# CookiePPP/cookietts

Hardware: AMD Instinct MI355X
Metric: audio samples/sec (22.05kHz) WaveGlow infer, 80×900 mel, 1/2/4/8 GPU; real-time factor (higher is better)
Workload: dtype f32; 1 GPU; WaveGlow full (12 flows, 512 WN ch, 8 groups, 8 layers) fp32 infer, batch 8 x (80x900) mel per GPU, sigma 0.6, random-init weights; batch_per_gpu=8, frames=900, parallelism=utterance-batch shard x1

## Files before the change

### cookietts_amd/_lib.py

```python
from __future__ import annotations

import ctypes as C
import os
import threading

import torch

from . import build as _build

_LOCK = threading.Lock()
_LIB = None


class WaveGlowConfig(C.Structure):
    _fields_ = [(n, C.c_int32) for n in (
        "n_mel_channels", "n_group", "n_flows", "n_early_every", "n_early_size",
        "win_length", "hop_length", "n_layers", "n_channels", "kernel_size", "cond_hidden", "speaker_embed_dim",
        "f32_gemm_mode")]


class StftConfig(C.Structure):
    _fields_ = [("filter_length", C.c_int32), ("hop_length", C.c_int32), ("win_length", C.c_int32),
                ("n_mel_channels", C.c_int32), ("clamp_val", C.c_float)]

# ... 253 lines not shown
    "ctts_waveflow_forward_f32": (C.c_int, [C.POINTER(WaveFlowConfig), _FP, _FP, _FP, _FP, C.c_float, C.c_int32, _FP, _FP, _FP, _FP,
                                            C.c_int32, C.c_int32, C.c_int32, _FP, C.c_size_t, _FP]),
    "ctts_waveflow_forward_cond_f32": (C.c_int, [C.POINTER(WaveFlowConfig), _FP, _FP, _FP, _FP, C.c_int32, C.c_int32, C.c_float,
                                                 C.c_int32, _FP, _FP, _FP, _FP, C.c_int32, C.c_int32, C.c_int32, _FP, C.c_size_t,
                                                 _FP]),
    "ctts_waveflow_abort_status": (C.c_int, [C.POINTER(WaveFlowConfig), C.c_int32, C.c_int32, _FP, C.c_size_t, _FP]),
    "ctts_wgax_packed_bytes": (C.c_size_t, [C.POINTER(WgaxConfig)]),
    "ctts_wgax_pack_flow": (C.c_int, [C.POINTER(WgaxConfig), C.c_int32, C.POINTER(WgaxFlowWeights), _FP, _FP]),
    "ctts_wgax_workspace_bytes": (C.c_size_t, [C.POINTER(WgaxConfig), C.c_int32, C.c_int64]),
    "ctts_wgax_inverse_f32": (C.c_int, [C.POINTER(WgaxConfig), _FP, _FP, _FP, C.c_int32, C.c_int32, C.c_int32, _FP,
                                        C.c_int32, C.c_int64, _FP, C.c_size_t, _FP]),
    "ctts_wgax_packed_f16_bytes": (C.c_size_t, [C.POINTER(WgaxConfig)]),
    "ctts_wgax_pack_flow_f16": (C.c_int, [C.POINTER(WgaxConfig), C.c_int32, C.POINTER(WgaxFlowWeights), _FP, _FP]),
    "ctts_wgax_workspace_f16_bytes": (C.c_size_t, [C.POINTER(WgaxConfig), C.c_int32, C.c_int64]),
    "ctts_wgax_inverse_f16": (C.c_int, [C.POINTER(WgaxConfig), _FP, _FP, _FP, C.c_int32, C.c_int32, C.c_int32, _FP,
                                        C.c_int32, C.c_int64, _FP, C.c_size_t, _FP]),
    "ctts_wgax_sep_packed_bytes": (C.c_size_t, [C.POINTER(WgaxConfig)]),
    "ctts_wgax_sep_pack_flow": (C.c_int, [C.POINTER(WgaxConfig), C.c_int32, C.POINTER(WgaxFlowWeights), C.POINTER(_FP),
                                          C.POINTER(_FP), _FP, _FP]),
    "ctts_wgax_sep_workspace_bytes": (C.c_size_t, [C.POINTER(WgaxConfig), C.c_int32, C.c_int64]),
    "ctts_wgax_sep_inverse_f32": (C.c_int, [C.POINTER(WgaxConfig), _FP, _FP, _FP, C.c_int32, C.c_int32, C.c_int32, _FP,
                                            C.c_int32, C.c_int64, _FP, C.c_size_t, _FP]),
    "ctts_depthwise_conv1d_f32": (C.c_int, [_FP, _FP, _FP, _FP] + [C.c_int32] * 7 + [_FP]),
    "ctts_hifigan_weight_floats": (C.c_size_t, [C.POINTER(HifiganConfig)]),
    "ctts_hifigan_packed_bytes": (C.c_size_t, [C.POINTER(HifiganConfig)]),
    "ctts_hifigan_pack_f32": (C.c_int, [C.POINTER(HifiganConfig), _FP, C.c_size_t, _FP, _FP]),
    "ctts_hifigan_workspace_bytes": (C.c_size_t, [C.POINTER(HifiganConfig), C.c_int32, C.c_int32]),
    "ctts_hifigan_forward_f32": (C.c_int, [C.POINTER(HifiganConfig), _FP, _FP, C.c_int32, _FP, C.c_int32, C.c_int32, _FP,
                                           C.c_size_t, _FP]),
    "ctts_hifigan_packed_f16_bytes": (C.c_size_t, [C.POINTER(HifiganConfig)]),
    "ctts_hifigan_pack_f16": (C.c_int, [C.POINTER(HifiganConfig), _FP, C.c_size_t, _FP, _FP]),
    "ctts_hifigan_workspace_f16_bytes": (C.c_size_t, [C.POINTER(HifiganConfig), C.c_int32, C.c_int32]),
    "ctts_hifigan_forward_f16": (C.c_int, [C.POINTER(HifiganConfig), _FP, _FP, C.c_int32, _FP, C.c_int32, C.c_int32, _FP,
                                           C.c_size_t, _FP]),
    "ctts_hifigan_packed_bf16x3_bytes": (C.c_size_t, [C.POINTER(HifiganConfig)]),
    "ctts_hifigan_pack_bf16x3": (C.c_int, [C.POINTER(HifiganConfig), _FP, C.c_size_t, _FP, _FP]),
    "ctts_hifigan_workspace_bf16x3_bytes": (C.c_size_t, [C.POINTER(HifiganConfig), C.c_int32, C.c_int32]),
    "ctts_hifigan_forward_bf16x3": (C.c_int, [C.POINTER(HifiganConfig), _FP, _FP, C.c_int32, _FP, C.c_int32, C.c_int32, _FP,
                                              C.c_size_t, _FP]),
    "ctts_replicate_halo_f32":(C.c_int, [_FP, C.c_int32, C.c_int32, C.c_int32, C.c_int32, C.c_int32, C.c_int32, _FP]),
    "ctts_embed_rows_f32": (C.c_int, [_FP, _FP, _FP, C.c_int32, C.c_int32, C.c_int32, C.c_int32, C.c_int32, C.c_int32,
                                      C.c_int32, _FP]),
    "ctts_scale_add_rows_f32": (C.c_int, [_FP, _FP, _FP, _FP, C.c_int32, C.c_int32, C.c_int32, C.c_int32, C.c_int32,
                                          _FP]),
    "ctts_deemphasis_f32": (C.c_int, [_FP, _FP, C.c_int32, C.c_int32, C.c_double, _FP]),
    "ctts_alignment_workspace_bytes": (C.c_size_t, [C.c_int32, C.c_int32, C.c_int32]),
    "ctts_alignment_metric_f32": (C.c_int, [_FP, _FP, _FP, C.c_int32, C.c_int32, C.c_int32, C.c_float, _FP, _FP,
                                            C.c_size_t, _FP]),
    "ctts_alignment_metric_masked_f32": (C.c_int, [_FP, _FP, _FP, _FP, C.c_int32, C.c_int32, C.c_int32, C.c_float, _FP, _FP,
                                                   C.c_size_t, _FP]),
    "ctts_first_over_thresh_f32": (C.c_int, [_FP, C.c_int32, C.c_int32, C.c_float, _FP, _FP]),
    "ctts_taco_loss_workspace_bytes": (C.c_size_t, [C.c_int32] * 4),
    "ctts_taco_loss_f32": (C.c_int, [C.POINTER(TacoLossParams)] + [_FP] * 13 + [C.c_int32] * 4 + [_FP, _FP, _FP, C.c_size_t,
                                                                                                  _FP]),
    "ctts_taco_loss_finalize_f32": (C.c_int, [C.POINTER(TacoLossParams)] + [_FP] * 9 + [C.c_int32] * 4 + [_FP, _FP, _FP,
                                                                                                          C.c_size_t, _FP]),
    "ctts_mel_error_packed_bytes": (C.c_size_t, [C.POINTER(MelErrorConfig)]),
    "ctts_mel_error_pack": (C.c_int, [C.POINTER(MelErrorConfig), C.c_int32, _FP, _FP, _FP, _FP]),
    "ctts_mel_error_workspace_bytes": (C.c_size_t, [C.POINTER(MelErrorConfig)] + [C.c_int32] * 3),
    "ctts_mel_error_f32": (C.c_int, [C.POINTER(MelErrorConfig)] + [_FP] * 6 + [C.c_int32] * 5 + [_FP] * 4 + [C.c_int32, _FP,
                                                                                                     C.c_size_t, _FP]),
    "ctts_mel_dtw_f32": (C.c_int, [_FP] * 6 + [C.c_int32] * 5 + [_FP]),
    "ctts_mel_dtw_generic_f32": (C.c_int, [_FP] * 6 + [C.c_int32] * 5 + [_FP]),
    "ctts_taco_stop_state_bytes": (C.c_size_t, [C.c_int32]),
    "ctts_taco_stop_reset": (C.c_int, [_FP, C.c_int32, C.c_int32, _FP]),
    "ctts_taco_stop_rule_f32": (C.c_int, [_FP, C.c_int32, C.c_int32, C.c_int32, C.c_int32, C.c_float, C.c_int32, _FP, _FP]),
    "ctts_retry_state_bytes": (C.c_size_t, [C.POINTER(RetryConfig)]),
    "ctts_retry_state_layout": (C.c_int, [C.POINTER(RetryConfig), C.POINTER(C.c_size_t)]),
    "ctts_retry_reset": (C.c_int, [C.POINTER(RetryConfig), _FP, _FP]),
    "ctts_retry_update_f32": (C.c_int, [C.POINTER(RetryConfig), _FP, _FP, _FP, _FP, _FP, _FP, C.c_int32, C.c_int32, _FP, _FP,
                                        _FP]),
    "ctts_retry_vocoder_batch_f32": (C.c_int, [C.POINTER(RetryConfig), _FP, _FP, C.c_int32, C.c_float, _FP]),
    "ctts_pcm16_concat": (C.c_int, [_FP, C.c_int32, _FP, C.c_int32, C.c_int64, C.c_int32, C.c_int32, _FP, C.c_int64, _FP,
                                    _FP]),
    "ctts_affine_rows_f32": (C.c_int, [_FP, C.c_int32, C.c_int32, C.c_int32, C.c_int32, C.c_int32, C.c_int32, C.c_float,
                                       C.c_float, _FP]),
    "ctts_vol_unscale_f32": (C.c_int, [_FP, C.c_int64, _FP]),
    "ctts_resample_rows_f32": (C.c_int, [_FP, _FP] + [C.c_int32] * 9 + [C.c_float, _FP]),
    "ctts_interleave_phases_f32": (C.c_int, [_FP, _FP] + [C.c_int32] * 10 + [_FP]),
    "ctts_last_gemm_loop": (C.c_int, []),
    "ctts_last_winograd_f43_width": (C.c_int, []),
    "ctts_tuning_reload": (C.c_int, []),
    "ctts_tuning_flags": (C.c_int, []),
    "ctts_profile_create": (C.c_int, [C.POINTER(C.c_void_p)]),
    "ctts_profile_bind": (C.c_int, [C.c_void_p]),
    "ctts_profile_collect": (C.c_int, [C.c_void_p, C.c_int32, C.POINTER(C.c_int64), C.POINTER(C.c_double)]),
    "ctts_profile_destroy": (C.c_int, [C.c_void_p]),
}

MODEL_GEMM_MODES = {None: 0, "default": 0, "f32": 1, "bf16x3": 2, "bf16x6": 3}
GEMM_MODES = {"f32": 1, "bf16x3": 2, "bf16x6": 3}
WG_OPT_COMPOSED_COND = 1


def model_gemm_mode(mode):
    try:
        return MODEL_GEMM_MODES[mode]
    except KeyError:
        raise ValueError(f"f32 GEMM mode {mode!r}: expected one of 'default', 'f32', 'bf16x3', 'bf16x6'") from None


def set_f32_gemm_mode(mode):
    if mode in (None, "default", "f32"):
        return "f32"
    raise RuntimeError(f"cookietts_amd.set_f32_gemm_mode({mode!r}): the process-wide default was removed; "
                       f"call model.set_f32_gemm_mode({mode!r}) on each model instead")


class Profile:

    def __init__(self):
        h = C.c_void_p()
        check(lib().ctts_profile_create(C.byref(h)), "ctts_profile_create")
        self._h = h

    def __enter__(self):
        check(lib().ctts_profile_bind(self._h), "ctts_profile_bind")
        return self

    def __exit__(self, *exc):
        check(lib().ctts_profile_bind(None), "ctts_profile_bind")
        return False

    bind = __enter__

    def unbind(self):
        self.__exit__()

    def collect(self, which):
        n, ms = C.c_int64(), C.c_double()
        check(lib().ctts_profile_collect(self._h, which, C.byref(n), C.byref(ms)), "ctts_profile_collect")
        return int(n.value), float(ms.value)

    def close(self):
        if self._h is not None and _LIB is not None:
            _LIB.ctts_profile_destroy(self._h)
        self._h = None

    def __del__(self):
        try:
            self.close()
        except Exception:
            pass


TUNING_BITS = {"CTTS_F32_NO_GLDS": 0, "CTTS_GEMM_NO_XCD_PAIR": 1, "CTTS_F32_WINOGRAD_FUSED_MIN": 2, "CTTS_BF16_NO_WIDE": 3, "CTTS_BF16_NO_PP": 4,
               "CTTS_F32_WINOGRAD_NO_FUSED": 5, "CTTS_F32_WINOGRAD_F43_MIN": 6, "CTTS_WF_NO_FUSE": 7,
               "CTTS_TACO_NO_FUSE": 8, "CTTS_F32_NO_SMALL": 9, "CTTS_F32_FORCE_SMALL": 10, "CTTS_F32_NO_SPLITK": 11, "CTTS_WF_NO_VEC_INTERP": 12,
               "CTTS_F32_NO_DEFER_SKIP": 13, "CTTS_WF_NO_REGION_SPLIT": 14, "CTTS_WF_NO_ROW_QUEUE": 15, "CTTS_WF_ROW_QUEUE_MIN": 16,
               "CTTS_WF_INJECT_ABORT": 17, "CTTS_WF_QUEUE_DEBUG": 18, "CTTS_F32_NO_ROUND_SPLIT": 19, "CTTS_BF16_PS": 20, "CTTS_BF16_NO_PS": 21,
               "CTTS_F32_WINOGRAD_NO_F43": 22,
               "CTTS_TACO_POLL_DELAY": 23, "CTTS_TACO_VALU": 24, "CTTS_UP_NO_MFMA": 25, "CTTS_F32_NO_WN_FOLD": 26, "CTTS_TACO_BG_NO_PIPE": 27,
               "CTTS_F32_NO_WINOGRAD": 28, "CTTS_F32_WINOGRAD_MIN": 29, "CTTS_F32_WINOGRAD_PLAIN": 30}
TUNING_BITS_EXT = {"CTTS_WF_FWD_ROWWISE": 31}


def tuning_reload():
    check(lib().ctts_tuning_reload(), "ctts_tuning_reload")


def tuning_active(name):
    bit = TUNING_BITS[name] if name in TUNING_BITS else TUNING_BITS_EXT[name]
    return bool(lib().ctts_tuning_flags() >> bit & 1)


PROF_WN_IN = 0
PROF_WN_RS = 1
PROF_WN_SKIP = 2
PROF_WN_IN0F = 3
PROF_WN_SKEND = 4
PROF_WN_RES_F = 5


class HipLibraryError(RuntimeError):
    pass


def lib_path():
    return _build.LIB_PATH


def lib():
    global _LIB
    if _LIB is not None:
        return _LIB
    with _LOCK:
        if _LIB is not None:
            return _LIB
        path = lib_path()
        if not os.path.exists(path):
            raise HipLibraryError(
                f"{path} is missing: build it with `python -m cookietts_amd.build` "
                "(or __graft_entry__.build()); there is no CPU fallback for the hot path")
        try:
            handle = C.CDLL(path)
        except OSError as e:
            raise HipLibraryError(f"cannot load {path}: {e}") from e
        for name, (res, args) in SIGNATURES.items():
            try:
                fn = getattr(handle, name)
            except AttributeError as e:
                raise HipLibraryError(f"{path} does not export {name}") from e
            fn.restype = res
            fn.argtypes = args
        if handle.ctts_abi_version() != 7:
            raise HipLibraryError(f"ABI version mismatch: library reports {handle.ctts_abi_version()}")
        _LIB = handle
    return _LIB


def last_error():
    msg = lib().ctts_last_error()
    return msg.decode(errors='replace') if msg else ''


def check(rc, what):
    if rc != 0:
        raise HipLibraryError(f"{what} failed (rc={rc}): {last_error()}")


def nbytes(fn, *args, what):
    n = fn(*args)
    if n == 0:
        raise HipLibraryError(f"{what}: {last_error()}")
    return n


def ptr(t):
    if t is None:
        return None
    return C.c_void_p(t.data_ptr())


def stream(device):
    return C.c_void_p(torch.cuda.current_stream(device).cuda_stream)
```

### cookietts_amd/csrc/gemm_f32.hip

```cpp
#include <atomic>
#include <cstdlib>
#include <mutex>

#include "gemm_f32.h"
#include "tuning.h"
#include "gemm_bf16.h"

namespace ctts {

typedef float f32x16 __attribute__((ext_vector_type(16)));

namespace {

constexpr int STAGE = GEMM_KC * (256 + 128);
constexpr int GEMM_GLDS_MAX_CHUNKS = 384;

__device__ __forceinline__ float fast_sigmoid(float u) {
    return __builtin_amdgcn_rcpf(1.0f + __builtin_amdgcn_exp2f(u * -1.4426950408889634f));
}
__device__ __forceinline__ float fast_tanh(float u) {
    return 1.0f - 2.0f * __builtin_amdgcn_rcpf(1.0f + __builtin_amdgcn_exp2f(u * 2.8853900817779268f));
}

typedef const __attribute__((address_space(1))) float* gfloat_ptr;
// ... 671 lines not shown
template <int EPI, bool GLDS>
void launch_shape_g(int bm, dim3 grid, hipStream_t stream, const GemmArgs& a) {
    const bool few = a.nseg <= 4;
    if (bm == 128) {
        if (few) hipLaunchKernelGGL((conv_gemm_f32_kernel<EPI, 1, 4, GLDS>), grid, dim3(256), 0, stream, a);
        else hipLaunchKernelGGL((conv_gemm_f32_kernel<EPI, 1, GEMM_MAX_SEG, GLDS>), grid, dim3(256), 0, stream, a);
    } else {
        if (few) hipLaunchKernelGGL((conv_gemm_f32_kernel<EPI, 2, 4, GLDS>), grid, dim3(256), 0, stream, a);
        else hipLaunchKernelGGL((conv_gemm_f32_kernel<EPI, 2, GEMM_MAX_SEG, GLDS>), grid, dim3(256), 0, stream, a);
    }
}

template <int EPI>
void launch_shape(int bm, dim3 grid, hipStream_t stream, const GemmArgs& a) {
    if (tuning().f32_no_glds || a.nch_total > GEMM_GLDS_MAX_CHUNKS) launch_shape_g<EPI, false>(bm, grid, stream, a);
    else if (gemm_split_level(a.gemm_mode) == 6) launch_shape_xs<EPI, 6>(bm, grid, stream, a);
    else if (gemm_split_level(a.gemm_mode) == 3) launch_shape_xs<EPI, 3>(bm, grid, stream, a);
    else launch_shape_g<EPI, true>(bm, grid, stream, a);
}

}

int get_gemm_f32_mode() { return gemm_f32_mode(); }
namespace { thread_local int t_last_loop = 0; }
void note_gemm_loop(int code) { t_last_loop = code; }
int last_gemm_loop() { return t_last_loop; }
int gemm_split_level(int m) {
    if (m == CTTS_GEMM_DEFAULT) m = gemm_f32_mode();
    if (m == CTTS_GEMM_BF16X3) return 3;
    if (m == CTTS_GEMM_BF16X6) return 6;
    return 0;
}
bool gemm_mode_is_split(int m) { return gemm_split_level(m) != 0; }

namespace {
std::mutex g_tune_mu;
Tuning g_tune{};
bool g_tune_loaded = false;
void load_tuning_locked() {
    auto on = [](const char* n) { return getenv(n) != nullptr; };
    auto num = [](const char* n, int d) { const char* v = getenv(n); return v ? atoi(v) : d; };
    g_tune.f32_no_glds = on("CTTS_F32_NO_GLDS");
    g_tune.f32_no_small = on("CTTS_F32_NO_SMALL");
    g_tune.f32_force_small = on("CTTS_F32_FORCE_SMALL");
    g_tune.f32_no_splitk = on("CTTS_F32_NO_SPLITK");
    g_tune.f32_no_round_split = on("CTTS_F32_NO_ROUND_SPLIT");
    g_tune.no_xcd_pair = on("CTTS_GEMM_NO_XCD_PAIR");
    g_tune.bf16_no_wide = on("CTTS_BF16_NO_WIDE");
    g_tune.bf16_no_pp = on("CTTS_BF16_NO_PP");
    g_tune.bf16_wide_min = num("CTTS_BF16_WIDE_MIN", 192);
    g_tune.bf16_ps = on("CTTS_BF16_PS");
    g_tune.bf16_no_ps = on("CTTS_BF16_NO_PS");
    g_tune.wf_no_fuse = on("CTTS_WF_NO_FUSE");
    g_tune.taco_no_fuse = on("CTTS_TACO_NO_FUSE");
    g_tune.taco_valu = on("CTTS_TACO_VALU");
    g_tune.up_no_mfma = on("CTTS_UP_NO_MFMA");
    g_tune.taco_bg_no_pipe = on("CTTS_TACO_BG_NO_PIPE");
    {
        static const int dflt[6] = {0x10000 | 36, 0x10000 | 96, 0x10000 | 12, 0x10000 | 20, 0x10000 | 8, 0x10000 | 8};
        int v[6];
        for (int i = 0; i < 6; ++i) v[i] = dflt[i];
        const char* e = getenv("CTTS_TACO_POLL_DELAY");
        if (e && sscanf(e, "%d,%d,%d,%d,%d,%d", v, v + 1, v + 2, v + 3, v + 4, v + 5) != 6)
            for (int i = 0; i < 6; ++i) v[i] = dflt[i];
        for (int i = 0; i < 6; ++i) g_tune.taco_poll_delay[i] = v[i] < 0 ? 0 : v[i];
        g_tune.taco_poll_delay_set = e != nullptr;
    }
    g_tune.wf_no_vec_interp = on("CTTS_WF_NO_VEC_INTERP");
    g_tune.wf_fwd_rowwise = on("CTTS_WF_FWD_ROWWISE");
    g_tune.wf_no_region_split = on("CTTS_WF_NO_REGION_SPLIT");
    g_tune.wf_no_row_queue = on("CTTS_WF_NO_ROW_QUEUE");
    g_tune.wf_row_queue_min = num("CTTS_WF_ROW_QUEUE_MIN", -1);
    g_tune.wf_inject_abort = num("CTTS_WF_INJECT_ABORT", 0);
    g_tune.wf_queue_debug = num("CTTS_WF_QUEUE_DEBUG", 0);
    g_tune.f32_no_defer_skip = on("CTTS_F32_NO_DEFER_SKIP");
    g_tune.f32_no_wn_fold = on("CTTS_F32_NO_WN_FOLD");
    g_tune.f32_no_winograd = on("CTTS_F32_NO_WINOGRAD");
    g_tune.f32_winograd_min = num("CTTS_F32_WINOGRAD_MIN", -1);
    g_tune.f32_winograd_plain = on("CTTS_F32_WINOGRAD_PLAIN");
    g_tune.f32_winograd_fused_min = num("CTTS_F32_WINOGRAD_FUSED_MIN", -1);
    g_tune.f32_winograd_no_fused = on("CTTS_F32_WINOGRAD_NO_FUSED");
    g_tune.f32_winograd_f43_min = num("CTTS_F32_WINOGRAD_F43_MIN", -1);
    g_tune.f32_winograd_no_f43 = on("CTTS_F32_WINOGRAD_NO_F43");
    g_tune.f32_cond_chain = on("CTTS_F32_COND_CHAIN");
    g_tune_loaded = true;
}
}

Tuning tuning() {
    std::lock_guard<std::mutex> lk(g_tune_mu);
    if (!g_tune_loaded) load_tuning_locked();
    return g_tune;
}
void reload_tuning() {
    std::lock_guard<std::mutex> lk(g_tune_mu);
    load_tuning_locked();
}

int gemm_check_args(int epi, const GemmArgs& a) {
    CTTS_CHECK_ARG(a.bm == 256 || a.bm == 128, "gemm: bm=%d", a.bm);
    CTTS_CHECK_ARG(gemm_mode_valid(a.gemm_mode), "gemm: f32_gemm_mode %d (0 default, 1 fp32 MFMA, 2 split bf16)", a.gemm_mode);
    const int bn = gemm_bn(a.bm);
    CTTS_CHECK_ARG(a.nseg >= 1 && a.nseg <= GEMM_MAX_SEG, "gemm: nseg=%d", a.nseg);
    int nch = 0;
    for (int s = 0; s < a.nseg; ++s) {
        CTTS_CHECK_ARG(a.seg[s].nch > 0 && a.seg[s].base, "gemm: empty segment %d", s);
        CTTS_CHECK_ARG(a.seg[s].shift >= -a.pad && a.seg[s].shift <= a.pad,
                       "gemm: shift %d exceeds halo %d", a.seg[s].shift, a.pad);
        nch += a.seg[s].nch;
    }
    CTTS_CHECK_ARG(nch == a.nch_total, "gemm: chunk count mismatch %d vs %d", nch, a.nch_total);
    if (a.interleave > 1) {
        CTTS_CHECK_ARG(a.interleave <= a.nseg, "gemm: interleave %d > nseg %d", a.interleave, a.nseg);
        for (int s = 1; s < a.interleave; ++s)
            CTTS_CHECK_ARG(a.seg[s].nch == a.seg[0].nch, "gemm: interleaved segments must have equal length");
    }
    CTTS_CHECK_ARG(a.a_nch_alloc == 0 || a.a_ch_off + a.nch_total <= a.a_nch_alloc, "gemm: A chunk window");
    CTTS_CHECK_ARG(a.ld % 4 == 0 && a.ntiles * bn + 2 * a.pad <= a.ld && a.L <= a.ntiles * bn,
                   "gemm: bad geometry ld=%d pad=%d L=%d ntiles=%d bn=%d", a.ld, a.pad, a.L, a.ntiles, bn);
    CTTS_CHECK_ARG(gemm_epi_is_pair(epi) || a.split % 32 == 0, "gemm: split %d not a multiple of 32", a.split);
    const int cpb = a.bm / 2;
    CTTS_CHECK_ARG(gemm_epi_is_pair(epi) ? (a.pairC > (a.MB - 1) * cpb && a.pairC <= a.MB * cpb)
                                         : (a.M > (a.MB - 1) * a.bm && a.M <= a.MB * a.bm),
                   "gemm: M=%d pairC=%d MB=%d bm=%d", a.M, a.pairC, a.MB, a.bm);
    CTTS_CHECK_ARG(a.dst_ld > 0 && a.dst0, "gemm: destination not set");
    CTTS_CHECK_ARG(a.addend_frames == 0 || ((epi == GEMM_EPI_GATE || epi == GEMM_EPI_GATEX) && a.addend && a.addend_frames <= a.addend_ld - a.addend_pad),
                   "gemm: interpolated addend needs the GATE epilogue (frames=%d)", a.addend_frames);
    CTTS_CHECK_ARG(a.gate >= 0 && a.gate < GATE_KINDS && (a.gate == 0 || epi == GEMM_EPI_GATE), "gemm: gate=%d with epilogue %d",
                   a.gate, epi);
    CTTS_CHECK_ARG((a.addend2 == nullptr && a.map_d == 0) ||
                       (epi == GEMM_EPI_GATE && a.gate == GATE_GTU && a.addend_frames == 0 && a.map_d >= 0 &&
                        (a.addend2 == nullptr || (a.addend && (a.addend2_sign == 1.0f || a.addend2_sign == -1.0f))) &&
                        (a.map_d == 0 || ((a.map_par == 0 || a.map_par == 1) && a.map_L > 0 && a.map_col0 >= 0))),
                   "gemm: second addend / mapped store need the GATE epilogue (epilogue %d, map_d=%d)", epi, a.map_d);
    CTTS_CHECK_ARG(epi != GEMM_EPI_GATE_RS ||
                       (a.bm == 128 && a.pairC <= 64 && a.MB == 1 && a.rs_wT && a.rs_bias && (a.rs_rows == 64 || a.rs_rows == 128)),
                   "gemm: fused res/skip needs bm=128, <= 64 channels, rs_wT / rs_bias and 64 or 128 res/skip rows");
    const int parts = a.parts > 1 ? a.parts : 1;
    CTTS_CHECK_ARG(a.parts >= 0 && a.parts <= 2 && (a.mseg == 0 || a.mseg == 2), "gemm: parts=%d mseg=%d", a.parts, a.mseg);
    if (parts > 1 || a.mseg) {
        CTTS_CHECK_ARG((epi == GEMM_EPI_SPLIT || (epi == GEMM_EPI_GATE && a.gate == GATE_GTU)) && a.bm == 256 && a.nseg <= 4 &&
                           a.interleave <= 1 && gemm_split_level(a.gemm_mode) == 0 && a.shape_blocks == 0 && a.addend_frames == 0,
                       "gemm: parts / mapped segment need the fp32 SPLIT or GATE launch of the 256-row shape (epilogue %d, nseg=%d)", epi, a.nseg);
        CTTS_CHECK_ARG(parts == 1 || epi != GEMM_EPI_SPLIT || (a.acc0 == 0 && a.src0 == nullptr && a.split >= a.M),
                       "gemm: a two-part SPLIT launch stores every row to dst0");
        CTTS_CHECK_ARG(parts == 1 || (long long)parts * a.ntiles * a.batch < (1ll << 31) / a.MB, "gemm: merged grid");
    }
    if (epi == GEMM_EPI_PHASE) {
        CTTS_CHECK_ARG(a.bm == 256 && a.nseg <= 4 && a.interleave <= 1 && gemm_split_level(a.gemm_mode) == 0 && parts == 1 && !a.mseg &&
                           a.shape_blocks == 0,
                       "gemm: the phase store needs the fp32 launch of the 256-row shape with <= 4 segments (nseg=%d)", a.nseg);
        CTTS_CHECK_ARG(a.phase >= 4 && a.phase <= 256 && (a.phase & (a.phase - 1)) == 0 && a.MB % a.phase == 0 && a.M == a.MB * a.bm,
                       "gemm: phase=%d MB=%d M=%d", a.phase, a.MB, a.M);
        CTTS_CHECK_ARG(a.dst_pad >= 0 && a.dst_pad % 4 == 0 && a.dst_ld % 4 == 0 && a.dst0_bstride % 4 == 0 &&
                           reinterpret_cast<uintptr_t>(a.dst0) % 16 == 0 && (long long)a.phase * a.L <= a.dst_ld - a.dst_pad,
                       "gemm: phase store dst_ld=%d dst_pad=%d phase=%d L=%d", a.dst_ld, a.dst_pad, a.phase, a.L);
    }
    if (a.mseg) {
        const GemmSeg& g = a.seg[1];
        CTTS_CHECK_ARG(epi == GEMM_EPI_GATE && a.nseg == 2 && a.map_d > 0 && a.map_d % 4 == 0 && a.map_col0 % 4 == 0 && a.mseg_pad >= 0 &&
                           a.mseg_pad % 4 == 0 && a.mseg_ld % 4 == 0 && a.mseg_ld - a.mseg_pad >= 4 && g.bstride % 4 == 0 &&
                           (parts == 1 || a.part_seg[1] % 4 == 0) && reinterpret_cast<uintptr_t>(g.base) % 16 == 0 && g.shift == 0 &&
                           g.mb_rows == 0,
                       "gemm: mapped segment d=%d col0=%d ld=%d pad=%d", a.map_d, a.map_col0, a.mseg_ld, a.mseg_pad);
    }
    return CTTS_OK;
// ... 119 lines not shown
```

### cookietts_amd/csrc/tuning.h

```cpp
#pragma once

namespace ctts {

struct Tuning {
    bool f32_no_glds;
    bool f32_no_small;
    bool f32_force_small;
    bool f32_no_splitk;
    bool f32_no_round_split;
    bool no_xcd_pair;
    bool bf16_no_wide;
    int bf16_wide_min;
    bool bf16_no_pp;
    bool bf16_ps;
    bool bf16_no_ps;
    bool wf_no_fuse;
    bool taco_poll_delay_set;
    int taco_poll_delay[6];
    bool taco_no_fuse;
    bool taco_bg_no_pipe;
    bool up_no_mfma;
    bool taco_valu;
    bool f32_no_defer_skip;
    bool f32_no_wn_fold;
    bool f32_no_winograd;
    int f32_winograd_min;
    bool f32_winograd_plain;
    int f32_winograd_fused_min;
    int f32_winograd_f43_min;
    bool f32_winograd_no_f43;
    bool f32_winograd_no_fused;
    bool f32_cond_chain;
    bool wf_no_region_split;
    bool wf_no_row_queue;
    int wf_row_queue_min;
    int wf_queue_debug;
    int wf_inject_abort;
    bool wf_fwd_rowwise;
    bool wf_no_vec_interp;
};

Tuning tuning();
void reload_tuning();

}
```

### cookietts_amd/csrc/waveglow_api.hip

```cpp
#include <mutex>
#include <vector>

#include "gemm_bf16.h"
#include "gemm_f32.h"
#include "tuning.h"
#include "waveglow_kernels.h"
#include "wn_winograd_layer.h"

namespace ctts {

static thread_local char g_err[512] = "";

void set_error(const char* fmt, ...) {
    va_list ap;
    va_start(ap, fmt);
    vsnprintf(g_err, sizeof(g_err), fmt, ap);
    va_end(ap);
}

namespace {

constexpr size_t ALIGN_F = 64;
inline size_t align_up(size_t v) { return (v + ALIGN_F - 1) / ALIGN_F * ALIGN_F; }
constexpr int A_TILE = GEMM_KC * GEMM_BM;

struct FlowDims { int n_rem, n_half, ch_off; };

struct Plan {
    ctts_waveglow_config c;
    int C, H, K0, n_in;
    int S;
    int nch0, nch1h, nch_in, nch_rs;
    int mb_in;
    int nch_in0f;
    std::vector<FlowDims> fd;
    size_t up_w, up_wp, up_b, cond0_A, cond0_b, cond1_A, cond1_b;
    size_t zero_b;
    bool up_mfma;
    bool cc;
    int ccP, ccJ, nch_cc;
    size_t cc_A, cc_b, cc_w10;
    struct Flow {
        size_t start_w, start_b, end_w, end_b, winv, spk_tab;
        std::vector<size_t> in_A, in_b, rs_A, rs_b;
        std::vector<size_t> res_A, res_b, skip_A, skip_b;
        size_t in0f_w, in0f_A, skend_W, skend_b;
        std::vector<size_t> wg_T2_A, wg_T3_A, wg_e_A, wg_o_A;
        size_t wg_dense;
        std::vector<size_t> wq_U_A[4], wq_e_A, wq_o_A;
    };
    std::vector<Flow> fl;
    size_t total;

    static constexpr int F32_SKIP_GROUP = 4;
    int mb_c() const { return (C + GEMM_BM - 1) / GEMM_BM; }
    int n_groups() const { return (c.n_layers + F32_SKIP_GROUP - 1) / F32_SKIP_GROUP; }
    int group_layers(int g) const { return g + 1 < n_groups() ? F32_SKIP_GROUP : c.n_layers - g * F32_SKIP_GROUP; }
    int rs_rows(int layer) const { return layer < c.n_layers - 1 ? 2 * C : C; }
    int rs_mb(int layer) const { return (rs_rows(layer) + GEMM_BM - 1) / GEMM_BM; }
};

int make_plan(const ctts_waveglow_config* cfg, Plan& p, int options = 0) {
    CTTS_CHECK_ARG(cfg != nullptr, "config is NULL");
    p.c = *cfg;
    CTTS_CHECK_ARG((options & ~CTTS_WG_OPT_COMPOSED_COND) == 0, "options=%d (CTTS_WG_OPT_*)", options);
    const bool want_cc = (options & CTTS_WG_OPT_COMPOSED_COND) != 0;
    const auto& c = p.c;
    CTTS_CHECK_ARG(c.n_flows >= 1 && c.n_layers >= 1 && c.n_layers <= 12, "n_flows=%d n_layers=%d", c.n_flows, c.n_layers);
    CTTS_CHECK_ARG(gemm_mode_valid(c.f32_gemm_mode), "f32_gemm_mode=%d (CTTS_GEMM_DEFAULT / _F32 / _BF16X3 / _BF16X6)", c.f32_gemm_mode);
    CTTS_CHECK_ARG(c.n_group >= 4 && c.n_group % 4 == 0 && c.n_group <= 16, "n_group=%d (4, 8, 12 or 16)", c.n_group);
    CTTS_CHECK_ARG(c.kernel_size == 3, "kernel_size=%d (only 3 built)", c.kernel_size);
    CTTS_CHECK_ARG(c.n_channels >= 128 && c.n_channels % 128 == 0, "n_channels=%d (multiple of 128)", c.n_channels);
    CTTS_CHECK_ARG(c.cond_hidden == GEMM_BM, "cond_hidden=%d (reference hard-codes 256)", c.cond_hidden);
    CTTS_CHECK_ARG(c.hop_length > 0 && c.win_length % c.hop_length == 0 && c.hop_length % c.n_group == 0,
                   "win=%d hop=%d n_group=%d", c.win_length, c.hop_length, c.n_group);
    CTTS_CHECK_ARG((c.n_mel_channels * c.n_group) % GEMM_KC == 0, "n_mel*n_group=%d not a multiple of 16",
                   c.n_mel_channels * c.n_group);
    CTTS_CHECK_ARG(c.n_early_every >= 1 && c.n_early_size >= 0 && c.n_early_size % 2 == 0, "early outputs");
    CTTS_CHECK_ARG(c.speaker_embed_dim >= 0 && c.speaker_embed_dim <= 1024, "speaker_embed_dim=%d", c.speaker_embed_dim);
    p.C = c.n_channels;
    p.H = c.cond_hidden;
    p.K0 = c.n_mel_channels * c.n_group;
    p.S = round_up(c.speaker_embed_dim, 32);
    CTTS_CHECK_ARG(p.S == 0 || p.K0 % 32 == 0, "multispeaker needs n_mel*n_group %% 32 == 0");
    p.nch0 = (p.K0 + p.S) / GEMM_KC;
    p.nch1h = p.H / GEMM_KC;
    p.nch_in = (c.kernel_size * p.C + p.H) / GEMM_KC;
    p.nch_rs = p.C / GEMM_KC;
    p.mb_in = 2 * p.C / GEMM_BM;
    p.nch_in0f = c.kernel_size + p.nch1h;
    int n_half = c.n_group / 2, n_rem = c.n_group;
    p.fd.resize(c.n_flows);
    for (int k = 0; k < c.n_flows; ++k) {
        if (k % c.n_early_every == 0 && k > 0) { n_half -= c.n_early_size / 2; n_rem -= c.n_early_size; }
        CTTS_CHECK_ARG(n_half >= 1 && n_rem == 2 * n_half, "flow %d: n_half=%d n_remaining=%d", k, n_half, n_rem);
        p.fd[k] = {n_rem, n_half, c.n_group - n_rem};
    }
    size_t o = 0;
    auto take = [&](size_t n) { size_t r = o; o = align_up(o + n); return r; };
    p.up_w = take((size_t)c.n_mel_channels * c.n_mel_channels * c.win_length);
    p.up_mfma = upsample_mfma_shape(c.n_mel_channels, c.win_length, c.hop_length, c.n_group);
    p.up_wp = p.up_mfma ? take((size_t)c.n_mel_channels * c.n_mel_channels * c.win_length) : 0;
    p.up_b = take(c.n_mel_channels);
    p.cond0_A = take((size_t)c.n_flows * p.nch0 * A_TILE);
    p.cond0_b = take((size_t)c.n_flows * GEMM_BM);
    p.cond1_A = take((size_t)c.n_flows * p.nch1h * A_TILE);
    p.cond1_b = take((size_t)c.n_flows * GEMM_BM);
    p.zero_b = take((size_t)p.mb_in * GEMM_BM);
    p.fl.resize(c.n_flows);
    for (int k = 0; k < c.n_flows; ++k) {
        auto& f = p.fl[k];
        f.start_w = take((size_t)p.C * p.fd[k].n_half);
        f.start_b = take(p.C);
        f.end_w = take((size_t)2 * p.fd[k].n_half * p.C);
        f.end_b = take(2 * p.fd[k].n_half);
        f.winv = take((size_t)p.fd[k].n_rem * p.fd[k].n_rem);
        f.spk_tab = take((size_t)CTTS_N_SPEAKERS * c.speaker_embed_dim);
        for (int i = 0; i < c.n_layers; ++i) {
            f.in_A.push_back(take((size_t)p.mb_in * p.nch_in * A_TILE));
            f.in_b.push_back(take((size_t)p.mb_in * GEMM_BM));
            f.rs_A.push_back(take((size_t)p.rs_mb(i) * p.nch_rs * A_TILE));
            f.rs_b.push_back(take((size_t)p.rs_mb(i) * GEMM_BM));
            f.res_A.push_back(i + 1 < c.n_layers ? take((size_t)p.mb_c() * p.nch_rs * A_TILE) : 0);
            f.res_b.push_back(i + 1 < c.n_layers ? take((size_t)p.mb_c() * GEMM_BM) : 0);
        }
        for (int gi = 0; gi < p.n_groups(); ++gi) {
            f.skip_A.push_back(take((size_t)p.mb_c() * p.group_layers(gi) * p.nch_rs * A_TILE));
            f.skip_b.push_back(take((size_t)p.mb_c() * GEMM_BM));
        }
        f.in0f_w = take((size_t)2 * p.C * FOLD_ROWS * c.kernel_size);
        f.in0f_A = take((size_t)p.mb_in * p.nch_in0f * A_TILE);
        f.skend_W = take((size_t)c.n_layers * p.C * 2 * p.fd[k].n_half);
        f.skend_b = take(2 * p.fd[k].n_half);
        for (int i = 0; i < c.n_layers; ++i) {
            f.wg_T2_A.push_back(take((size_t)p.mb_in * p.nch_rs * A_TILE));
            f.wg_T3_A.push_back(take((size_t)p.mb_in * p.nch_rs * A_TILE));
            f.wg_e_A.push_back(take((size_t)p.mb_in * (p.nch_rs + p.nch1h) * A_TILE));
            f.wg_o_A.push_back(take((size_t)p.mb_in * (p.nch_rs + p.nch1h) * A_TILE));
        }
        const bool f43 = wn_winograd_layer_f43_supported(p.C, p.H);
        for (int i = 0; f43 && i < c.n_layers; ++i) {
            for (auto& u : f.wq_U_A) u.push_back(take((size_t)p.mb_in * p.nch_rs * A_TILE));
            f.wq_e_A.push_back(take((size_t)p.mb_in * (p.nch_rs + p.nch1h) * A_TILE));
            f.wq_o_A.push_back(take((size_t)p.mb_in * (p.nch_rs + p.nch1h) * A_TILE));
        }
        f.wg_dense = take((size_t)(f43 ? 6 : 3) * 2 * p.C * p.C);
    }
    p.ccP = c.hop_length / c.n_group;
    p.ccJ = c.win_length / c.hop_length;
    p.nch_cc = p.ccJ * c.n_mel_channels / GEMM_KC;
    p.cc = want_cc && p.S == 0 && c.n_mel_channels % GEMM_KC == 0 && p.ccJ >= 1 && p.ccJ <= 4 && p.ccP >= 4 && p.ccP <= GEMM_BM &&
           (p.ccP & (p.ccP - 1)) == 0;
    p.cc_A = p.cc_b = p.cc_w10 = 0;
    if (p.cc) {
        p.cc_A = take((size_t)c.n_flows * p.ccP * p.nch_cc * A_TILE);
        p.cc_b = take((size_t)c.n_flows * p.ccP * GEMM_BM);
        p.cc_w10 = take((size_t)c.n_flows * 2 * p.H * p.K0);
    }
    p.total = o;
    return CTTS_OK;
}

struct Geom { int L, ld, pad, ntiles; };

int make_geom(const Plan& p, int frames, Geom& g) {
    CTTS_CHECK_ARG(frames >= 1, "frames=%d", frames);
    const long long T = (long long)frames * p.c.hop_length;
    g.L = (int)(T / p.c.n_group);
    int maxd = 1 << (p.c.n_layers - 1);
    g.pad = round_up(maxd > 128 ? maxd : 128, 32);
    g.ntiles = (g.L + GEMM_BN - 1) / GEMM_BN;
    g.ld = round_up(g.L, 256) + 2 * g.pad;
    return CTTS_OK;
}

struct PairGeom { int d, Lp, ntiles; };
PairGeom pair_geom(const Geom& g, int layer) {
    const int d = 1 << layer;
    const int Lp = (g.L + 2 * d - 1) / (2 * d) * d;
    return {d, Lp, (Lp + GEMM_BN - 1) / GEMM_BN};
}
int pair_ld(const Plan& p, const Geom& g) {
    int nt = 0;
    for (int i = 0; i < p.c.n_layers; ++i) nt = std::max(nt, pair_geom(g, i).ntiles);
    return nt * GEMM_BN;
}
PairGeom quad_geom(const Geom& g, int layer) {
    const int d = 1 << layer;
    const int Lq = (g.L + 4 * d - 1) / (4 * d) * d;
    return {d, Lq, (Lq + 63) / 64};
}
int quad_ld(const Plan& p, const Geom& g) {
    int nt = 0;
    for (int i = 0; i < p.c.n_layers; ++i) nt = std::max(nt, quad_geom(g, i).ntiles);
    return round_up(nt * 64, 128);
}
enum class InForm { Direct, WinogradSeparate, WinogradPaired, WinogradLayer, WinogradLayerF43 };

constexpr long long WINOGRAD_MIN_COLS = 28800;
constexpr long long WINOGRAD_FUSED_MIN_COLS = 28800;
constexpr long long WINOGRAD_F43_MIN_COLS = 28800;

InForm in_form(const Plan& p, const Geom& g, const Tuning& t) {
    auto long_enough = [&](int knob, long long cols) { return (long long)g.L >= (knob >= 0 ? knob : cols); };
    if (t.f32_no_winograd || gemm_split_level(p.c.f32_gemm_mode) != 0 || !long_enough(t.f32_winograd_min, WINOGRAD_MIN_COLS))
        return InForm::Direct;
    if (t.f32_winograd_plain || !gemm_f32_dma_staged(p.nch_rs + p.nch1h)) return InForm::WinogradSeparate;
    if (t.f32_winograd_no_fused || t.f32_no_glds || !wn_winograd_layer_supported(p.C, p.H) ||
        !long_enough(t.f32_winograd_fused_min, WINOGRAD_FUSED_MIN_COLS))
        return InForm::WinogradPaired;
    if (t.f32_winograd_no_f43 || !wn_winograd_layer_f43_supported(p.C, p.H) || !long_enough(t.f32_winograd_f43_min, WINOGRAD_F43_MIN_COLS))
        return InForm::WinogradLayer;
    return InForm::WinogradLayerF43;
}

bool cond_composed(const Plan& p, int frames, const Tuning& t) {
    if (!p.cc || t.f32_cond_chain || gemm_split_level(p.c.f32_gemm_mode) != 0) return false;
    const long long tiles_f = (frames + GEMM_BN - 1) / GEMM_BN, tiles_l = ((long long)frames * p.ccP + GEMM_BN - 1) / GEMM_BN;
    return tiles_f * p.ccP * p.ccJ * p.c.n_mel_channels < tiles_l * (p.K0 + p.H);
}
struct MelGeom { int ntiles, pad, ld; };
MelGeom mel_geom(int frames) {
    const int nt = (frames + GEMM_BN - 1) / GEMM_BN;
    return {nt, 4, nt * GEMM_BN + 8};
}

struct Workspace {
    float *audio, *spect, *spk, *h_tmp, *h_all, *x, *act, *out;
    float* melp;
    float* act_all;
    float* a16;
    float* skend;
    float *wgV, *wgT, *wgH;
    int ldp, ldq;
    size_t total;
};

void carve(const Plan& p, const Geom& g, int batch, float* base, InForm in, bool composed, Workspace& w) {
    size_t o = 0;
    auto take = [&](size_t n) { size_t r = o; o = align_up(o + n); return base ? base + r : nullptr; };
    const size_t B = batch;
    w.audio = take(B * p.c.n_group * g.L);
    w.spect = composed ? nullptr : take(B * p.K0 * g.ld);
    w.melp = composed ? take(B * p.c.n_mel_channels * mel_geom(g.L / p.ccP).ld) : nullptr;
    w.spk = take(B * p.c.n_flows * p.S * g.ld);
    w.h_tmp = composed ? nullptr : take(B * p.c.n_flows * p.H * g.ld);
    w.h_all = take(B * p.c.n_flows * p.H * g.ld);
    w.x = take(B * p.C * g.ld);
    w.act = take(B * p.C * g.ld);
    w.out = take(B * p.C * g.ld);
    w.act_all = take((size_t)std::min(p.c.n_layers, (int)Plan::F32_SKIP_GROUP) * B * p.C * g.ld);
    w.a16 = take(B * FOLD_ROWS * g.ld);
    w.skend = take(B * p.c.n_group * g.ld);
    w.wgV = w.wgT = w.wgH = nullptr;
    w.ldp = w.ldq = 0;
    if (in != InForm::Direct) {
        w.ldp = pair_ld(p, g);
        w.ldq = in == InForm::WinogradLayerF43 ? quad_ld(p, g) : 0;
        w.wgV = take(std::max((size_t)4 * w.ldp, (size_t)6 * w.ldq) * B * p.C);
        w.wgT = take((size_t)2 * B * 2 * p.C * w.ldp);
        w.wgH = take(std::max((size_t)2 * w.ldp, (size_t)4 * w.ldq) * B * p.H);
    }
    w.total = o;
}

struct Prof {
    std::mutex mu;
    std::vector<std::pair<hipEvent_t, hipEvent_t>> ev[CTTS_PROF_N];
    std::vector<std::pair<hipEvent_t, hipEvent_t>> pool;
};
thread_local Prof* t_prof = nullptr;

struct ProfScope {
    int which; hipStream_t s; hipEvent_t stop = nullptr; bool active = false;
    ProfScope(int which_, hipStream_t s_) : which(which_), s(s_) {
        Prof* pr = t_prof;
        if (!pr) return;
        std::lock_guard<std::mutex> lk(pr->mu);
        std::pair<hipEvent_t, hipEvent_t> e;
        if (!pr->pool.empty()) { e = pr->pool.back(); pr->pool.pop_back(); }
        else { if (hipEventCreate(&e.first) != hipSuccess || hipEventCreate(&e.second) != hipSuccess) return; }
        (void)hipEventRecord(e.first, s);
        stop = e.second;
        pr->ev[which].push_back(e);
        active = true;
    }
    ~ProfScope() { if (active) (void)hipEventRecord(stop, s); }
};

__global__ __launch_bounds__(256) void speaker_rows_kernel(const float* __restrict__ table, const int64_t* __restrict__ ids,
                                                           float* __restrict__ spk, int k, int n_flows, int S, int sdim,
                                                           int L, int ld, int pad) {
    const int n = blockIdx.x * 256 + threadIdx.x;
    const int e = blockIdx.y, b = blockIdx.z;
    if (n >= ld) return;
    float v = 0.f;
    if (e < sdim && n >= pad && n < pad + L) {
        const long long id = ids[b];
        v = (id >= 0 && id < CTTS_N_SPEAKERS) ? table[(size_t)id * sdim + e] : __builtin_nanf("");
    }
    spk[((size_t)b * n_flows * S + (size_t)k * S + e) * ld + n] = v;
}


__global__ __launch_bounds__(256) void cond_compose_w10_kernel(const float* __restrict__ w1, const float* __restrict__ w0,
                                                               double* __restrict__ w10, int H, int K0) {
    const int c = blockIdx.x * 256 + threadIdx.x, r = blockIdx.y;
    if (c >= K0) return;
    double s = 0.0;
    for (int h = 0; h < H; ++h) s += (double)w1[(size_t)r * H + h] * (double)w0[(size_t)h * K0 + c];
    w10[(size_t)r * K0 + c] = s;
}

__global__ __launch_bounds__(GEMM_BM) void cond_compose_A_kernel(const double* __restrict__ w10, const float* __restrict__ up_w,
                                                                 float* __restrict__ A, int n_mel, int G, int hop, int win, int P,
                                                                 int nch) {
    const int rl = threadIdx.x, kidx = blockIdx.x, m = blockIdx.y;
    const int r = m * (GEMM_BM / P) + rl / P, p = rl % P;
    const int j = kidx / n_mel, ci = kidx % n_mel;
    const float* u = up_w + (size_t)ci * n_mel * win + hop * j + G * p;
    const double* wr = w10 + (size_t)r * n_mel * G;
    double s = 0.0;
    for (int co = 0; co < n_mel; ++co)
        for (int q = 0; q < G; ++q) s += wr[co * G + q] * (double)u[(size_t)co * win + q];
    A[(((size_t)m * nch + kidx / GEMM_KC) * GEMM_KC + kidx % GEMM_KC) * GEMM_BM + rl] = (float)s;
}

__global__ __launch_bounds__(GEMM_BM) void cond_compose_bias_kernel(const float* __restrict__ w0, const float* __restrict__ b0,
                                                                    const float* __restrict__ w1, const float* __restrict__ b1,
                                                                    const float* __restrict__ up_b, float* __restrict__ bias, int K0,
                                                                    int G, int P) {
    __shared__ double t0[GEMM_BM];
    const int r = threadIdx.x;
    double s = b0[r];
    for (int c = 0; c < K0; ++c) s += (double)w0[(size_t)r * K0 + c] * (double)up_b[c / G];
    t0[r] = s;
    __syncthreads();
    s = b1[r];
    for (int h = 0; h < GEMM_BM; ++h) s += (double)w1[(size_t)r * GEMM_BM + h] * t0[h];
    const int HR = GEMM_BM / P;
    for (int p = 0; p < P; ++p) bias[(size_t)(r / HR) * GEMM_BM + (r % HR) * P + p] = (float)s;
}

__global__ __launch_bounds__(256) void mel_pad_kernel(const float* __restrict__ mel, float* __restrict__ melp, int frames, int ld, int pad) {
    const int n = blockIdx.x * 256 + threadIdx.x;
    const size_t row = (size_t)blockIdx.z * gridDim.y + blockIdx.y;
    if (n >= ld) return;
    const int f = n - pad;
    melp[row * ld + n] = f >= 0 && f < frames ? mel[row * frames + f] : 0.0f;
}

size_t fwd_mix_off(const Plan& p, int k) {
    size_t o = 0;
    for (int j = 0; j < k; ++j) o += align_up((size_t)p.fd[j].n_rem * p.fd[j].n_rem);
    return o;
}
int fwd_log_s_rows(const Plan& p, int k) {
    int r = 0;
    for (int j = 0; j < k; ++j) r += p.fd[j].n_half;
    return r;
}

struct FwdSums { double *ls_part, *z_part; int nblk_ls, nblk_z; size_t total; };

void carve_fwd(const Plan& p, const Geom& g, int batch, float* base, InForm in, bool composed, Workspace& w, FwdSums& f) {
    carve(p, g, batch, base, in, composed, w);
    f.nblk_ls = (g.L + 255) / 256;
    f.nblk_z = (int)(((long long)p.c.n_group * g.L + FWD_SUMSQ_CHUNK - 1) / FWD_SUMSQ_CHUNK);
    size_t o = w.total;
    auto take = [&](size_t doubles) { size_t r = o; o = align_up(o + 2 * doubles); return base ? reinterpret_cast<double*>(base + r) : nullptr; };
    f.ls_part = take((size_t)batch * p.c.n_flows * f.nblk_ls);
    f.z_part = take((size_t)batch * f.nblk_z);
    f.total = o;
}

int workspace_fits(const char* what, size_t have, size_t need) {
    if (need <= have) return CTTS_OK;
    set_error("%s: workspace %zu bytes < required %zu", what, have, need);
    return CTTS_E_WORKSPACE;
}

enum class StackForm { PerLayer, Deferred, Folded };

struct WnCall {
    Plan p; Geom g; Tuning t;
    const float* blob = nullptr;
    int batch = 0, frames = 0;
    hipStream_t s = nullptr;
    Workspace w{};
    FwdSums sums{};
    long long cstride = 0, hstride = 0;
    StackForm stack = StackForm::PerLayer;
    InForm in = InForm::Direct;
    bool composed = false;
    float* audio = nullptr;
    const float* h_all = nullptr;

    int begin(const ctts_waveglow_config* cfg, const void* packed, int batch_, int frames_, void* stream, int options = 0) {
        int rc = make_plan(cfg, p, options); if (rc) return rc;
        rc = make_geom(p, frames_, g); if (rc) return rc;
        t = tuning();
        blob = static_cast<const float*>(packed); batch = batch_; frames = frames_; s = as_stream(stream);
        cstride = (long long)p.C * g.ld;
        hstride = (long long)p.c.n_flows * p.H * g.ld;
        return CTTS_OK;
    }
    int take_workspace(const char* what, void* workspace, size_t workspace_bytes, bool forward) {
        in = in_form(p, g, t);
        stack = t.f32_no_defer_skip ? StackForm::PerLayer : t.f32_no_wn_fold ? StackForm::Deferred : StackForm::Folded;
        composed = cond_composed(p, frames, t);
        if (forward) carve_fwd(p, g, batch, static_cast<float*>(workspace), in, composed, w, sums);
        else carve(p, g, batch, static_cast<float*>(workspace), in, composed, w);
        audio = w.audio; h_all = w.h_all;
        return workspace_fits(what, workspace_bytes, (forward ? sums.total : w.total) * sizeof(float));
    }

    const float* h(int k) const { return h_all + (size_t)k * p.H * g.ld; }
    size_t act_stride() const { return (size_t)batch * p.C * g.ld; }
    float* act(int i) const { return stack == StackForm::PerLayer ? w.act : w.act_all + (size_t)(i % Plan::F32_SKIP_GROUP) * act_stride(); }
    bool group_ends(int i) const { return i == p.c.n_layers - 1 || (i + 1) % Plan::F32_SKIP_GROUP == 0; }
    bool in_place(int i) const { return in != InForm::WinogradSeparate && (1 << i) % 4 == 0; }
    size_t plane(int rows) const { return (size_t)batch * rows * w.ldp; }

    GemmArgs header() const {
        GemmArgs a{};
        a.gemm_mode = p.c.f32_gemm_mode;
        a.ld = g.ld; a.pad = g.pad; a.L = g.L; a.ntiles = g.ntiles; a.batch = batch;
        a.dst_ld = g.ld; a.dst_pad = g.pad;
        return a;
    }
    GemmArgs in_gemm(int k, int i) const {
        const auto& f = p.fl[k];
        const bool fold0 = stack == StackForm::Folded && i == 0;
        const int dil = 1 << i, nch = fold0 ? 1 : p.nch_rs;
        const float* taps = fold0 ? w.a16 : w.x;
        const long long tstride = fold0 ? (long long)FOLD_ROWS * g.ld : cstride;
        GemmArgs a = header();
        a.A = blob + (fold0 ? f.in0f_A : f.in_A[i]); a.bias = blob + f.in_b[i];
        a.nseg = 4; a.interleave = 3; a.nch_total = fold0 ? p.nch_in0f : p.nch_in; a.MB = p.mb_in;
        for (int tap = 0; tap < 3; ++tap) a.seg[tap] = {taps, tstride, nch, (tap - 1) * dil, 0, 0};
        a.seg[3] = {h(k), hstride, p.nch1h, 0, 0, 0};
        a.dst0 = act(i); a.dst0_bstride = cstride;
        a.M = 2 * p.C; a.pairC = p.C;
        return a;
    }
    GemmArgs behind(size_t A, size_t bias, int rows, const float* acts, int n, int split, bool acc1) const {
        GemmArgs a = header();
        a.A = blob + A; a.bias = blob + bias;
        a.nseg = n; a.nch_total = n * p.nch_rs; a.MB = (rows + GEMM_BM - 1) / GEMM_BM;
        for (int j = 0; j < n; ++j) a.seg[j] = {acts + (size_t)j * act_stride(), cstride, p.nch_rs, 0, 0, 0};
        a.M = rows; a.split = split;
        a.dst0 = w.x; a.dst0_bstride = cstride; a.acc0 = 1;
        a.dst1 = w.out; a.dst1_bstride = cstride; a.acc1 = acc1 ? 1 : 0;
        return a;
    }
    GemmArgs res(int k, int i) const { return behind(p.fl[k].res_A[i], p.fl[k].res_b[i], p.C, act(i), 1, p.C, false); }
    GemmArgs skip_group(int k, int gi) const { return behind(p.fl[k].skip_A[gi], p.fl[k].skip_b[gi], p.C, w.act_all, p.group_layers(gi), 0, gi > 0); }
    GemmArgs res_skip(int k, int i) const {
        return behind(p.fl[k].rs_A[i], p.fl[k].rs_b[i], p.rs_rows(i), act(i), 1, i == p.c.n_layers - 1 ? 0 : p.C, i > 0);
    }
    GemmArgs cond0(const float* spect, const float* spk, float* h_tmp) const {
        GemmArgs a = header();
        a.A = blob + p.cond0_A; a.bias = blob + p.cond0_b;
        a.nseg = 1; a.nch_total = p.nch0; a.MB = p.c.n_flows;
        a.seg[0] = {spect, (long long)p.K0 * g.ld, p.K0 / GEMM_KC, 0, 0, 0};
        if (p.S) {
            a.nseg = 2;
            a.seg[1] = {spk, (long long)p.c.n_flows * p.S * g.ld, p.S / GEMM_KC, 0, p.S, 0};
        }
        a.dst0 = h_tmp; a.dst0_bstride = hstride; a.acc0 = 0;
        a.dst1 = h_tmp; a.dst1_bstride = hstride; a.acc1 = 0;
        a.split = p.c.n_flows * GEMM_BM;
        a.M = p.c.n_flows * GEMM_BM;
        return a;
    }
    GemmArgs cond1(const float* spect, const float* spk, float* h_tmp, float* h_out) const {
        GemmArgs a = cond0(spect, spk, h_tmp);
        a.A = blob + p.cond1_A; a.bias = blob + p.cond1_b;
        a.nseg = 1; a.nch_total = p.nch1h;
        a.seg[0] = {h_tmp, hstride, p.nch1h, 0, GEMM_BM, 0};
        a.dst0 = h_out; a.dst1 = h_out;
        return a;
    }
    GemmArgs cond_composed_gemm(const float* melp, float* h_out) const {
        const MelGeom mg = mel_geom(frames);
        GemmArgs a{};
        a.gemm_mode = p.c.f32_gemm_mode;
        a.ld = mg.ld; a.pad = mg.pad; a.L = frames; a.ntiles = mg.ntiles; a.batch = batch;
        a.A = blob + p.cc_A; a.bias = blob + p.cc_b;
        a.nseg = p.ccJ; a.nch_total = p.nch_cc; a.MB = p.c.n_flows * p.ccP;
        for (int j = 0; j < p.ccJ; ++j)
            a.seg[j] = {melp, (long long)p.c.n_mel_channels * mg.ld, p.c.n_mel_channels / GEMM_KC, -j, 0, 0};
        a.M = a.MB * GEMM_BM; a.split = a.M;
        a.phase = p.ccP;
        a.dst0 = h_out; a.dst0_bstride = hstride; a.dst_ld = g.ld; a.dst_pad = g.pad;
        return a;
    }
    GemmArgs wg_header(int i) const {
        const PairGeom pg = pair_geom(g, i);
        GemmArgs a{};
        a.gemm_mode = p.c.f32_gemm_mode;
        a.ld = w.ldp; a.pad = 0; a.L = pg.Lp; a.ntiles = pg.ntiles; a.batch = batch; a.MB = p.mb_in;
        a.M = 2 * p.C;
        if (in == InForm::WinogradPaired) a.parts = 2;
        return a;
    }
    GemmArgs wg_T(int k, int i, int j) const {
        const auto& f = p.fl[k];
        GemmArgs a = wg_header(i);
        a.A = blob + (j == 0 ? f.wg_T2_A[i] : f.wg_T3_A[i]); a.bias = blob + p.zero_b;
        a.nseg = 1; a.nch_total = p.nch_rs;
        a.seg[0] = {w.wgV + (1 + j) * plane(p.C), (long long)p.C * w.ldp, p.nch_rs, 0, 0, 0};
        a.split = 2 * p.C;
        a.dst0 = w.wgT + j * plane(2 * p.C); a.dst0_bstride = (long long)2 * p.C * w.ldp; a.dst_ld = w.ldp; a.dst_pad = 0;
        if (a.parts == 2) {
            a.part_A = (long long)f.wg_T3_A[i] - (long long)f.wg_T2_A[i];
            a.part_seg[0] = (long long)plane(p.C);
            a.part_dst0 = (long long)plane(2 * p.C);
        }
        return a;
    }
    GemmArgs wg_gate(int k, int i, int j) const {
        const auto& f = p.fl[k];
        GemmArgs a = wg_header(i);
        a.A = blob + (j == 0 ? f.wg_e_A[i] : f.wg_o_A[i]); a.bias = blob + f.in_b[i];
        a.nseg = 2; a.nch_total = p.nch_rs + p.nch1h;
        a.seg[0] = {w.wgV + (j == 0 ? 0 : 3) * plane(p.C), (long long)p.C * w.ldp, p.nch_rs, 0, 0, 0};
        if (in_place(i)) {
            a.seg[1] = {h(k), hstride, p.nch1h, 0, 0, 0};
            a.mseg = 2; a.mseg_ld = g.ld; a.mseg_pad = g.pad;
        } else {
            a.seg[1] = {w.wgH + j * plane(p.H), (long long)p.H * w.ldp, p.nch1h, 0, 0, 0};
        }
        a.split = 0; a.pairC = p.C;
        a.dst0 = act(i); a.dst0_bstride = cstride; a.dst_ld = g.ld; a.dst_pad = g.pad;
        a.addend = w.wgT; a.addend2 = w.wgT + plane(2 * p.C); a.addend_bstride = (long long)2 * p.C * w.ldp;
        a.addend2_sign = j == 0 ? 1.0f : -1.0f;
        a.map_d = 1 << i; a.map_L = g.L; a.map_par = j;
        if (a.parts == 2) {
            a.part_A = (long long)f.wg_o_A[i] - (long long)f.wg_e_A[i];
            a.part_seg[0] = (long long)(3 * plane(p.C));
            a.part_seg[1] = in_place(i) ? 0 : (long long)plane(p.H);
        }
        return a;
    }
    WnWinogradLayerArgs wg_layer(int k, int i) const {
        const auto& f = p.fl[k];
        const bool f43 = in == InForm::WinogradLayerF43;
        const PairGeom sg = f43 ? quad_geom(g, i) : pair_geom(g, i);
        const int ldw = f43 ? w.ldq : w.ldp;
        WnWinogradLayerArgs a{};
        if (f43) {
            a.form = WNWG_F43;
            a.A_T2 = blob + f.wq_U_A[0][i]; a.A_T3 = blob + f.wq_U_A[1][i]; a.A_T4 = blob + f.wq_U_A[2][i]; a.A_T5 = blob + f.wq_U_A[3][i];
            a.A_e = blob + f.wq_e_A[i]; a.A_o = blob + f.wq_o_A[i];
        } else {
            a.A_T2 = blob + f.wg_T2_A[i]; a.A_T3 = blob + f.wg_T3_A[i]; a.A_e = blob + f.wg_e_A[i]; a.A_o = blob + f.wg_o_A[i];
        }
        a.bias = blob + f.in_b[i];
        a.V = w.wgV; a.vplane = (long long)batch * p.C * ldw;
        a.Hc = w.wgH; a.hplane = (long long)batch * p.H * ldw;
        a.h2 = h(k); a.h_bstride = hstride;
        a.act = act(i); a.act_bstride = cstride;
        a.C = p.C; a.H = p.H; a.batch = batch;
        a.ldp = ldw; a.Lp = sg.Lp; a.ntiles = sg.ntiles;
        a.d = sg.d; a.L = g.L; a.ld = g.ld; a.pad = g.pad;
        a.in_place = in_place(i);
        return a;
    }

    int gemm(int prof_slot, int epi, const GemmArgs& a) const {
        ProfScope ps(prof_slot, s);
        return launch_gemm_f32(epi, a, s);
    }
    int wg_transform(int k, int i) const {
        if (in == InForm::WinogradLayerF43) {
            const PairGeom qg = quad_geom(g, i);
            const int ncols = t.f32_no_small ? round_up(qg.ntiles * 64, 128) : qg.ntiles * 64;
            return launch_winograd_transform_quad(w.x, cstride, h(k), hstride, w.wgV, w.wgH, batch, p.C, p.H, qg.d, g.L, qg.Lp, g.ld, g.pad,
                                                  w.ldq, ncols, !in_place(i), s);
        }
        const PairGeom pg = pair_geom(g, i);
        return launch_winograd_transform(w.x, cstride, h(k), hstride, w.wgV, w.wgH, batch, p.C, p.H, pg.d, g.L, pg.Lp, g.ld, g.pad, w.ldp,
                                         pg.ntiles * GEMM_BN, !in_place(i), in != InForm::WinogradSeparate, s);
    }
    int in_layer(int k, int i) const {
        ProfScope ps(CTTS_PROF_WN_IN, s);
        if (stack == StackForm::Folded && i == 0) return gemm(CTTS_PROF_WN_IN0F, GEMM_EPI_GATE, in_gemm(k, i));
        int rc = in == InForm::Direct ? CTTS_OK : wg_transform(k, i);
        if (rc) return rc;
        switch (in) {
        case InForm::Direct:
            return launch_gemm_f32(GEMM_EPI_GATE, in_gemm(k, i), s);
        case InForm::WinogradLayer:
        case InForm::WinogradLayerF43:
            return launch_wn_winograd_layer(wg_layer(k, i), s);
        case InForm::WinogradSeparate:
        case InForm::WinogradPaired:
            const int np = in == InForm::WinogradPaired ? 1 : 2;
            for (int j = 0; j < np; ++j)
                if ((rc = launch_gemm_f32(GEMM_EPI_SPLIT, wg_T(k, i, j), s))) return rc;
            for (int j = 0; j < np; ++j)
                if ((rc = launch_gemm_f32(GEMM_EPI_GATE, wg_gate(k, i, j), s))) return rc;
        }
        return rc;
    }
    int start(int k, const float* a_in) const {
        const auto& f = p.fl[k];
        const auto& d = p.fd[k];
        return launch_wn_start(a_in, blob + f.start_w, blob + f.start_b, w.x, batch, p.C, p.c.n_group, d.ch_off, d.n_half, g.L, g.ld, g.pad, s);
    }
    int skip_end(int k, int gi, bool tail, float* wave, const CouplingForward* fwd) const {
        const auto& f = p.fl[k];
        const auto& d = p.fd[k];
        ProfScope ps(CTTS_PROF_WN_SKEND, s);
        return launch_skip_end(w.act_all, (long long)act_stride(), p.group_layers(gi),
                               blob + f.skend_W + (size_t)gi * Plan::F32_SKIP_GROUP * p.C * 2 * d.n_half, w.skend, gi == 0, tail,
                               blob + f.skend_b, blob + f.winv, audio, wave, batch, p.C, p.c.n_group, d.ch_off, d.n_half, g.L, g.ld,
                               g.pad, s, tail ? fwd : nullptr);
    }
    int flow_tail(int k, const float* out, float* a_io, float* wave, const CouplingForward* fwd) const {
        const auto& f = p.fl[k];
        const auto& d = p.fd[k];
        return launch_flow_tail(out, a_io, wave, blob + f.end_w, blob + f.end_b, blob + f.winv, batch, p.C, p.c.n_group, d.ch_off,
                                d.n_half, g.L, g.ld, g.pad, s, fwd);
    }

    int flow_folded(int k, float* wave, const CouplingForward* fwd) const {
        const auto& d = p.fd[k];
        int rc = start(k, audio);
        if (rc) return rc;
        if ((rc = launch_wn_start_ones(audio, w.a16, batch, p.c.n_group, d.ch_off, d.n_half, g.L, g.ld, g.pad, s))) return rc;
        for (int i = 0; i < p.c.n_layers; ++i) {
            const bool last = i == p.c.n_layers - 1;
            if ((rc = in_layer(k, i))) return rc;
            if (!last && (rc = gemm(CTTS_PROF_WN_RES_F, GEMM_EPI_SPLIT, res(k, i)))) return rc;
            if (group_ends(i) && (rc = skip_end(k, i / Plan::F32_SKIP_GROUP, last, wave, fwd))) return rc;
        }
        return CTTS_OK;
    }
    int stack_deferred(int k, const float* a_in) const {
        int rc = start(k, a_in);
        if (rc) return rc;
        for (int i = 0; i < p.c.n_layers; ++i) {
            if ((rc = in_layer(k, i))) return rc;
            if (i < p.c.n_layers - 1 && (rc = gemm(CTTS_PROF_WN_RS, GEMM_EPI_SPLIT, res(k, i)))) return rc;
            if (group_ends(i) && (rc = gemm(CTTS_PROF_WN_SKIP, GEMM_EPI_SPLIT, skip_group(k, i / Plan::F32_SKIP_GROUP)))) return rc;
        }
        return CTTS_OK;
    }
    int stack_per_layer(int k, const float* a_in) const {
        int rc = start(k, a_in);
        if (rc) return rc;
        for (int i = 0; i < p.c.n_layers; ++i) {
            if ((rc = in_layer(k, i))) return rc;
            if ((rc = gemm(CTTS_PROF_WN_RS, GEMM_EPI_SPLIT, res_skip(k, i)))) return rc;
        }
        return CTTS_OK;
    }
    int run_flow(int k, float* wave, const CouplingForward* fwd) const {
        if (stack == StackForm::Folded) return flow_folded(k, wave, fwd);
        const int rc = stack == StackForm::Deferred ? stack_deferred(k, audio) : stack_per_layer(k, audio);
        return rc ? rc : flow_tail(k, w.out, audio, wave, fwd);
    }
    int run_flow_forward(const float* fwd_blob, int k, const float* wave, float* log_s_flow, long long ls_bstride) const {
        const auto& d = p.fd[k];
        int rc = launch_flow_head_forward(fwd_blob + fwd_mix_off(p, k), wave, audio, batch, p.c.n_group, d.ch_off, d.n_rem, g.L, s);
        if (rc) return rc;
        const CouplingForward cf{log_s_flow, ls_bstride, sums.ls_part + (size_t)k * sums.nblk_ls, (long long)p.c.n_flows * sums.nblk_ls};
        return run_flow(k, nullptr, &cf);
    }

    int upsample(const float* mel, float* spect) const {
        return launch_upsample_squeeze(mel, blob + p.up_w, p.up_mfma ? blob + p.up_wp : nullptr, blob + p.up_b, spect, batch,
                                       p.c.n_mel_channels, frames, p.c.win_length, p.c.hop_length, p.c.n_group, g.ld, g.pad, s);
    }
    int speaker_rows(const int64_t* ids, float* spk) const {
        if (p.S == 0) return CTTS_OK;
// ... 376 lines not shown
    CTTS_CHECK_ARG(w && packed, "pack_flow: NULL pointer");
    hipStream_t s = as_stream(stream);
    float* blob = static_cast<float*>(packed);
    const auto& f = p.fl[k];
    const auto& d = p.fd[k];
    const int C = p.C, H = p.H, ks = p.c.kernel_size;
    auto d2d = [&](size_t off, const float* src, size_t n) -> int {
        CTTS_CHECK_ARG(src != nullptr, "pack_flow: NULL weight pointer");
        CTTS_CHECK_HIP(hipMemcpyAsync(blob + off, src, n * sizeof(float), hipMemcpyDeviceToDevice, s));
        return CTTS_OK;
    };
    if ((rc = d2d(f.start_w, w->start_w, (size_t)C * d.n_half))) return rc;
    if ((rc = d2d(f.start_b, w->start_b, C))) return rc;
    if ((rc = d2d(f.end_w, w->end_w, (size_t)2 * d.n_half * C))) return rc;
    if ((rc = d2d(f.end_b, w->end_b, 2 * d.n_half))) return rc;
    if ((rc = d2d(f.winv, w->w_inverse, (size_t)d.n_rem * d.n_rem))) return rc;
    CTTS_CHECK_ARG(w->cond_w[0] && w->cond_w[1] && w->cond_w[2] && w->cond_b[0] && w->cond_b[1] && w->cond_b[2],
                   "pack_flow: NULL cond weights");
    const int sdim = p.c.speaker_embed_dim;
    if ((rc = launch_pack_a(blob + p.cond0_A + (size_t)k * p.nch0 * A_TILE, w->cond_w[0], GEMM_BM, 1, p.nch0, 0, p.K0,
                            GEMM_EPI_SPLIT, C, H, 0, p.K0 + sdim, 1, s))) return rc;
    if (sdim) {
        if ((rc = launch_pack_a(blob + p.cond0_A + (size_t)k * p.nch0 * A_TILE, w->cond_w[0] + p.K0, GEMM_BM, 1, p.nch0,
                                p.K0, sdim, GEMM_EPI_SPLIT, C, H, 0, p.K0 + sdim, 1, s))) return rc;
        if ((rc = d2d(f.spk_tab, w->speaker_embed, (size_t)CTTS_N_SPEAKERS * sdim))) return rc;
    }
    if ((rc = launch_pack_bias(blob + p.cond0_b + (size_t)k * GEMM_BM, GEMM_BM, 1, w->cond_b[0], 0, nullptr, 0,
                               GEMM_EPI_SPLIT, C, H, s))) return rc;
    if ((rc = launch_pack_a(blob + p.cond1_A + (size_t)k * p.nch1h * A_TILE, w->cond_w[1], GEMM_BM, 1, p.nch1h, 0, H,
                            GEMM_EPI_SPLIT, C, H, 0, H, 1, s))) return rc;
    if ((rc = launch_pack_bias(blob + p.cond1_b + (size_t)k * GEMM_BM, GEMM_BM, 1, w->cond_b[1], 0, nullptr, 0,
                               GEMM_EPI_SPLIT, C, H, s))) return rc;
    for (int i = 0; i < p.c.n_layers; ++i) {
        CTTS_CHECK_ARG(w->in_w[i] && w->in_b[i] && w->rs_w[i] && w->rs_b[i], "pack_flow: NULL layer %d weights", i);
        for (int t = 0; t < ks; ++t)
            if ((rc = launch_pack_a(blob + f.in_A[i], w->in_w[i] + t, GEMM_BM, p.mb_in, p.nch_in, 0, C, GEMM_EPI_GATE, C,
                                    2 * C, 0, (long long)C * ks, ks, s, ks, t))) return rc;
        if ((rc = launch_pack_a(blob + f.in_A[i], w->cond_w[2], GEMM_BM, p.mb_in, p.nch_in, ks * C, H, GEMM_EPI_GATE, C,
                                2 * C, (long long)2 * C * i, H, 1, s))) return rc;
        if ((rc = launch_pack_bias(blob + f.in_b[i], GEMM_BM, p.mb_in, w->in_b[i], 0, w->cond_b[2], (long long)2 * C * i,
                                   GEMM_EPI_GATE, C, 2 * C, s))) return rc;
        const int rows = p.rs_rows(i);
        if ((rc = launch_pack_a(blob + f.rs_A[i], w->rs_w[i], GEMM_BM, p.rs_mb(i), p.nch_rs, 0, C, GEMM_EPI_SPLIT, C, rows,
                                0, C, 1, s))) return rc;
        if ((rc = launch_pack_bias(blob + f.rs_b[i], GEMM_BM, p.rs_mb(i), w->rs_b[i], 0, nullptr, 0, GEMM_EPI_SPLIT, C, rows,
                                   s))) return rc;
        const bool last = i == p.c.n_layers - 1;
        const int gi = i / Plan::F32_SKIP_GROUP, gj = i % Plan::F32_SKIP_GROUP;
        if (!last) {
            if ((rc = launch_pack_a(blob + f.res_A[i], w->rs_w[i], GEMM_BM, p.mb_c(), p.nch_rs, 0, C, GEMM_EPI_SPLIT, C, C,
                                    0, C, 1, s))) return rc;
            if ((rc = launch_pack_bias(blob + f.res_b[i], GEMM_BM, p.mb_c(), w->rs_b[i], 0, nullptr, 0, GEMM_EPI_SPLIT, C, C,
                                       s))) return rc;
        }
        if ((rc = launch_pack_a(blob + f.skip_A[gi], w->rs_w[i], GEMM_BM, p.mb_c(), p.group_layers(gi) * p.nch_rs, gj * C, C,
                                GEMM_EPI_SPLIT, C, C, last ? 0 : C, C, 1, s))) return rc;
        hipLaunchKernelGGL(skip_bias_kernel, dim3((p.mb_c() * GEMM_BM + 255) / 256), dim3(256), 0, s, blob + f.skip_b[gi],
                           w->rs_b[i] + (last ? 0 : C), C, p.mb_c() * GEMM_BM, gj == 0 ? 1 : 0);
        CTTS_CHECK_LAUNCH("skip_bias_f32");
    }
    auto pack_gate = [&](size_t A, const float* U, long long u_ld, int u_step, int i) -> int {
        const int nch = p.nch_rs + p.nch1h;
        const int rc = launch_pack_a(blob + A, U, GEMM_BM, p.mb_in, nch, 0, C, GEMM_EPI_GATE, C, 2 * C, 0, u_ld, u_step, s);
        return rc ? rc : launch_pack_a(blob + A, w->cond_w[2], GEMM_BM, p.mb_in, nch, C, H, GEMM_EPI_GATE, C, 2 * C, (long long)2 * C * i, H, 1, s);
    };
    for (int i = 0; i < p.c.n_layers; ++i) {
        float* dense = blob + f.wg_dense;
        const size_t dn = (size_t)2 * C * C;
        if ((rc = launch_winograd_g(w->in_w[i], dense, 2 * C, C, s))) return rc;
        if ((rc = launch_pack_a(blob + f.wg_T2_A[i], dense, GEMM_BM, p.mb_in, p.nch_rs, 0, C, GEMM_EPI_SPLIT, C, 2 * C, 0, C, 1, s))) return rc;
        if ((rc = launch_pack_a(blob + f.wg_T3_A[i], dense + dn, GEMM_BM, p.mb_in, p.nch_rs, 0, C, GEMM_EPI_SPLIT, C, 2 * C, 0, C, 1, s))) return rc;
        if ((rc = pack_gate(f.wg_e_A[i], w->in_w[i], (long long)C * ks, ks, i))) return rc;
        if ((rc = pack_gate(f.wg_o_A[i], dense + 2 * dn, C, 1, i))) return rc;
    }
    for (int i = 0; i < (f.wq_e_A.empty() ? 0 : p.c.n_layers); ++i) {
        float* dense = blob + f.wg_dense;
        const size_t dn = (size_t)2 * C * C;
        if ((rc = launch_winograd_g43(w->in_w[i], dense, 2 * C, C, s))) return rc;
        for (int j = 0; j < 4; ++j)
            if ((rc = launch_pack_a(blob + f.wq_U_A[j][i], dense + (1 + j) * dn, GEMM_BM, p.mb_in, p.nch_rs, 0, C, GEMM_EPI_SPLIT, C, 2 * C, 0, C, 1, s))) return rc;
        if ((rc = pack_gate(f.wq_e_A[i], dense, C, 1, i))) return rc;
        if ((rc = pack_gate(f.wq_o_A[i], dense + 5 * dn, C, 1, i))) return rc;
    }
    if ((rc = launch_fold_in0(w->in_w[0], w->start_w, w->start_b, blob + f.in0f_w, C, d.n_half, ks, s))) return rc;
    for (int t = 0; t < ks; ++t)
        if ((rc = launch_pack_a(blob + f.in0f_A, blob + f.in0f_w + t, GEMM_BM, p.mb_in, p.nch_in0f, 0, FOLD_ROWS, GEMM_EPI_GATE, C,
                                2 * C, 0, (long long)FOLD_ROWS * ks, ks, s, ks, t))) return rc;
    if ((rc = launch_pack_a(blob + f.in0f_A, w->cond_w[2], GEMM_BM, p.mb_in, p.nch_in0f, ks * FOLD_ROWS, H, GEMM_EPI_GATE, C,
                            2 * C, 0, H, 1, s))) return rc;
    return launch_fold_skend(w->rs_w, w->rs_b, w->end_w, w->end_b, blob + f.skend_W, blob + f.skend_b, C, p.c.n_layers, d.n_half, s);
}

size_t ctts_waveglow_packed_bytes_opt(const ctts_waveglow_config* cfg, int32_t options) {
    Plan p;
    if (make_plan(cfg, p, options)) return 0;
    return p.total * sizeof(float);
}

int ctts_waveglow_has_composed_cond(const ctts_waveglow_config* cfg) {
    Plan p;
    return make_plan(cfg, p, CTTS_WG_OPT_COMPOSED_COND) == CTTS_OK && p.cc ? 1 : 0;
}

int ctts_waveglow_pack_cond_composed(const ctts_waveglow_config* cfg, int32_t k, const ctts_waveglow_flow_weights* w, void* packed,
                                     void* stream) {
    Plan p;
    int rc = make_plan(cfg, p, CTTS_WG_OPT_COMPOSED_COND); if (rc) return rc;
    CTTS_CHECK_ARG(p.cc, "pack_cond_composed: this config has no composed conditioning (ctts_waveglow_has_composed_cond)");
    CTTS_CHECK_ARG(k >= 0 && k < p.c.n_flows, "pack_cond_composed: flow %d", k);
    CTTS_CHECK_ARG(w && packed && w->cond_w[0] && w->cond_w[1] && w->cond_b[0] && w->cond_b[1], "pack_cond_composed: NULL pointer");
    hipStream_t s = as_stream(stream);
    float* blob = static_cast<float*>(packed);
    const int H = p.H;
    double* w10 = reinterpret_cast<double*>(blob + p.cc_w10) + (size_t)k * H * p.K0;
    hipLaunchKernelGGL(cond_compose_w10_kernel, dim3((p.K0 + 255) / 256, H), dim3(256), 0, s, w->cond_w[1], w->cond_w[0], w10, H, p.K0);
    hipLaunchKernelGGL(cond_compose_A_kernel, dim3(p.ccJ * p.c.n_mel_channels, p.ccP), dim3(GEMM_BM), 0, s, w10, blob + p.up_w,
                       blob + p.cc_A + (size_t)k * p.ccP * p.nch_cc * A_TILE, p.c.n_mel_channels, p.c.n_group, p.c.hop_length,
                       p.c.win_length, p.ccP, p.nch_cc);
    hipLaunchKernelGGL(cond_compose_bias_kernel, dim3(1), dim3(GEMM_BM), 0, s, w->cond_w[0], w->cond_b[0], w->cond_w[1], w->cond_b[1],
                       blob + p.up_b, blob + p.cc_b + (size_t)k * p.ccP * GEMM_BM, p.K0, p.c.n_group, p.ccP);
    CTTS_CHECK_LAUNCH("cond_compose");
    return CTTS_OK;
}

size_t ctts_waveglow_workspace_bytes(const ctts_waveglow_config* cfg, int32_t batch, int32_t frames) {
    return ctts_waveglow_workspace_bytes_opt(cfg, batch, frames, 0);
}

size_t ctts_waveglow_workspace_bytes_opt(const ctts_waveglow_config* cfg, int32_t batch, int32_t frames, int32_t options) {
    Plan p; Geom g; Workspace w;
    if (make_plan(cfg, p, options) || make_geom(p, frames, g) || batch < 1) return 0;
    const Tuning t = tuning();
    carve(p, g, batch, nullptr, in_form(p, g, t), cond_composed(p, frames, t), w);
    return w.total * sizeof(float);
}

int ctts_upsample_squeeze_f32(const ctts_waveglow_config* cfg, const void* packed, const float* mel, float* spect,
                              int32_t batch, int32_t frames, void* stream) {
    WnCall c;
    const int rc = c.begin(cfg, packed, batch, frames, stream); if (rc) return rc;
    CTTS_CHECK_ARG(packed && mel && spect && batch >= 1, "upsample_squeeze: bad argument");
    return c.upsample(mel, spect);
}

int ctts_wn_cond_f32(const ctts_waveglow_config* cfg, const void* packed, const float* spect, const float* spk_rows,
                     float* h_tmp, float* h_all, int32_t batch, int32_t frames, void* stream) {
    WnCall c;
    const int rc = c.begin(cfg, packed, batch, frames, stream); if (rc) return rc;
    CTTS_CHECK_ARG(packed && spect && h_tmp && h_all && batch >= 1, "wn_cond: bad argument");
    return c.cond(spect, spk_rows, h_tmp, h_all);
}

size_t ctts_wn_cond_composed_scratch_bytes(const ctts_waveglow_config* cfg, int32_t batch, int32_t frames) {
    Plan p;
    if (make_plan(cfg, p, CTTS_WG_OPT_COMPOSED_COND) || !p.cc || batch < 1 || frames < 1) return 0;
    return (size_t)batch * p.c.n_mel_channels * mel_geom(frames).ld * sizeof(float);
}

int ctts_wn_cond_composed_f32(const ctts_waveglow_config* cfg, const void* packed, const float* mel, float* scratch, float* h_all,
                              int32_t batch, int32_t frames, void* stream) {
    WnCall c;
    const int rc = c.begin(cfg, packed, batch, frames, stream, CTTS_WG_OPT_COMPOSED_COND); if (rc) return rc;
    CTTS_CHECK_ARG(packed && mel && scratch && h_all && batch >= 1, "wn_cond_composed: bad argument");
    return c.cond_from_mel(mel, scratch, h_all);
}

// ... 53 lines not shown
    if (batch < 1) { set_error("forward_workspace_bytes: batch=%d", batch); return 0; }
    const Tuning t = tuning();
    carve_fwd(p, g, batch, nullptr, in_form(p, g, t), cond_composed(p, frames, t), w, f);
    return f.total * sizeof(float);
}

int ctts_waveglow_flow_forward_f32(const ctts_waveglow_config* cfg, const void* packed, const void* packed_fwd, int32_t flow,
                                   float* z, const float* wave, const float* h_all, float* log_s, double* sum_log_s,
                                   int32_t batch, int32_t frames, void* workspace, size_t workspace_bytes, void* stream) {
    WnCall c;
    int rc = c.begin(cfg, packed, batch, frames, stream); if (rc) return rc;
    CTTS_CHECK_ARG(flow >= 0 && flow < c.p.c.n_flows, "waveglow_flow_forward: flow %d", flow);
    CTTS_CHECK_ARG(packed && packed_fwd && z && h_all && workspace && batch >= 1, "waveglow_flow_forward: bad argument");
    CTTS_CHECK_ARG(wave == nullptr || flow == 0, "waveglow_flow_forward: only flow 0 reads the waveform (flow %d)", flow);
    if ((rc = c.take_workspace("waveglow_flow_forward", workspace, workspace_bytes, true))) return rc;
    c.audio = z; c.h_all = h_all;
    rc = c.run_flow_forward(static_cast<const float*>(packed_fwd), flow, wave, log_s, (long long)c.p.fd[flow].n_half * c.g.L);
    if (rc || !sum_log_s) return rc;
    const FwdSums& f = c.sums;
    return launch_sum_partials(f.ls_part + (size_t)flow * f.nblk_ls, (long long)c.p.c.n_flows * f.nblk_ls, 0, f.nblk_ls, sum_log_s, 1, 1,
                               batch, c.s);
}

int ctts_waveglow_forward_spk_f32(const ctts_waveglow_config* cfg, const void* packed, const void* packed_fwd, const float* mel,
                                  const float* audio, const int64_t* speaker_ids, float* z, float* log_s, double* sums,
                                  int32_t batch, int32_t frames, void* workspace, size_t workspace_bytes, void* stream) {
    WnCall c;
    int rc = c.begin(cfg, packed, batch, frames, stream); if (rc) return rc;
    const Plan& p = c.p;
    CTTS_CHECK_ARG(packed && packed_fwd && mel && audio && z && workspace && batch >= 1, "forward: bad argument");
    CTTS_CHECK_ARG(p.S == 0 || speaker_ids != nullptr, "multispeaker model (speaker_embed_dim=%d) needs speaker ids (glow.py:193)",
                   p.c.speaker_embed_dim);
    if ((rc = c.take_workspace("forward", workspace, workspace_bytes, true))) return rc;
    c.audio = z;
    if ((rc = c.conditioning(mel, speaker_ids))) return rc;
    const int L = c.g.L, S = fwd_log_s_rows(p, p.c.n_flows);
    for (int k = 0; k < p.c.n_flows; ++k) {
        float* ls = log_s ? log_s + (size_t)fwd_log_s_rows(p, k) * L : nullptr;
        rc = c.run_flow_forward(static_cast<const float*>(packed_fwd), k, k == 0 ? audio : nullptr, ls, (long long)S * L);
        if (rc) return rc;
    }
    if (!sums) return CTTS_OK;
    const FwdSums& f = c.sums;
    rc = launch_sum_partials(f.ls_part, (long long)p.c.n_flows * f.nblk_ls, f.nblk_ls, f.nblk_ls, sums, p.c.n_flows + 1, p.c.n_flows,
                             batch, c.s);
    if (rc) return rc;
    rc = launch_sumsq_partials(z, f.z_part, batch, (long long)p.c.n_group * L, f.nblk_z, c.s);
    if (rc) return rc;
    return launch_sum_partials(f.z_part, f.nblk_z, 0, f.nblk_z, sums + p.c.n_flows, p.c.n_flows + 1, 1, batch, c.s);
}

int ctts_waveglow_infer_f32(const ctts_waveglow_config* cfg, const void* packed, const float* mel,
                            const float* z_scaled, float* wave, int32_t batch, int32_t frames, void* workspace,
                            size_t workspace_bytes, void* stream) {
    return ctts_waveglow_infer_spk_f32(cfg, packed, mel, z_scaled, nullptr, wave, batch, frames, workspace,
                                       workspace_bytes, stream);
}

int ctts_waveglow_infer_spk_f32(const ctts_waveglow_config* cfg, const void* packed, const float* mel,
                                const float* z_scaled, const int64_t* speaker_ids, float* wave, int32_t batch,
                                int32_t frames, void* workspace, size_t workspace_bytes, void* stream) {
    return ctts_waveglow_infer_spk_f32_opt(cfg, packed, mel, z_scaled, speaker_ids, wave, batch, frames, workspace, workspace_bytes, 0,
                                           stream);
}

int ctts_waveglow_infer_spk_f32_opt(const ctts_waveglow_config* cfg, const void* packed, const float* mel,
                                    const float* z_scaled, const int64_t* speaker_ids, float* wave, int32_t batch,
                                    int32_t frames, void* workspace, size_t workspace_bytes, int32_t options, void* stream) {
    WnCall c;
    int rc = c.begin(cfg, packed, batch, frames, stream, options); if (rc) return rc;
    CTTS_CHECK_ARG(packed && mel && z_scaled && wave && workspace && batch >= 1, "infer: bad argument");
    if ((rc = c.take_workspace("infer", workspace, workspace_bytes, false))) return rc;
    CTTS_CHECK_HIP(hipMemcpyAsync(c.audio, z_scaled, (size_t)batch * c.p.c.n_group * c.g.L * sizeof(float), hipMemcpyDeviceToDevice, c.s));
    if ((rc = c.conditioning(mel, speaker_ids))) return rc;
    for (int k = c.p.c.n_flows - 1; k >= 0; --k)
        if ((rc = c.run_flow(k, k == 0 ? wave : nullptr, nullptr))) return rc;
    return CTTS_OK;
}


int ctts_last_gemm_loop(void) { return last_gemm_loop(); }
int ctts_last_winograd_f43_width(void) { return last_wn_winograd_f43_width(); }
int ctts_tuning_reload(void) { reload_tuning(); return CTTS_OK; }
int ctts_tuning_flags(void) {
    const Tuning t = tuning();
    return (t.f32_no_glds ? 1 : 0) | (t.no_xcd_pair ? 2 : 0) | (t.bf16_no_wide ? 8 : 0) | (t.bf16_no_pp ? 16 : 0) |
           (t.wf_no_fuse ? 128 : 0) | (t.taco_no_fuse ? 256 : 0) | (t.f32_no_small ? 512 : 0) | (t.f32_force_small ? 1024 : 0) |
           (t.f32_no_splitk ? 2048 : 0) | (t.wf_no_vec_interp ? 4096 : 0) | (t.f32_no_defer_skip ? 8192 : 0) |
           (t.wf_no_region_split ? 16384 : 0) | (t.wf_no_row_queue ? 32768 : 0) | (t.wf_row_queue_min >= 0 ? 65536 : 0) |
           (t.wf_inject_abort ? 131072 : 0) | (t.wf_queue_debug ? 262144 : 0) | (t.f32_no_round_split ? 524288 : 0) |
           (t.bf16_ps ? (1 << 20) : 0) | (t.bf16_no_ps ? (1 << 21) : 0) | (t.taco_poll_delay_set ? (1 << 23) : 0) |
           (t.taco_valu ? (1 << 24) : 0) | (t.up_no_mfma ? (1 << 25) : 0) | (t.f32_no_wn_fold ? (1 << 26) : 0) |
           (t.taco_bg_no_pipe ? (1 << 27) : 0) | (t.f32_no_winograd ? (1 << 28) : 0) | (t.f32_winograd_min >= 0 ? (1 << 29) : 0) |
           (t.f32_winograd_plain ? (1 << 30) : 0) | (t.f32_winograd_fused_min >= 0 ? 4 : 0) | (t.f32_winograd_no_fused ? 32 : 0) |
           (t.f32_winograd_f43_min >= 0 ? (1 << 6) : 0) | (t.f32_winograd_no_f43 ? (1 << 22) : 0) |
           (t.wf_fwd_rowwise ? (int)(1u << 31) : 0);
}

int ctts_profile_create(void** handle) {
    CTTS_CHECK_ARG(handle, "profile_create: NULL");
    *handle = new Prof();
    return CTTS_OK;
}

int ctts_profile_bind(void* handle) {
    t_prof = static_cast<Prof*>(handle);
    return CTTS_OK;
}

int ctts_profile_collect(void* handle, int32_t which, int64_t* launches, double* total_ms) {
    Prof* pr = static_cast<Prof*>(handle);
    CTTS_CHECK_ARG(pr && which >= 0 && which < CTTS_PROF_N && launches && total_ms, "profile_collect: bad argument");
    std::lock_guard<std::mutex> lk(pr->mu);
    double tot = 0.0;
    int64_t n = 0;
    for (auto& e : pr->ev[which]) {
        float ms = 0.f;
        CTTS_CHECK_HIP(hipEventSynchronize(e.second));
        CTTS_CHECK_HIP(hipEventElapsedTime(&ms, e.first, e.second));
        tot += ms; ++n;
        pr->pool.push_back(e);
    }
    pr->ev[which].clear();
    *launches = n; *total_ms = tot;
    return CTTS_OK;
}

int ctts_profile_destroy(void* handle) {
    Prof* pr = static_cast<Prof*>(handle);
    if (!pr) return CTTS_OK;
    if (t_prof == pr) t_prof = nullptr;
    {
        std::lock_guard<std::mutex> lk(pr->mu);
        for (int w = 0; w < CTTS_PROF_N; ++w)
            for (auto& e : pr->ev[w]) { (void)hipEventDestroy(e.first); (void)hipEventDestroy(e.second); }
        for (auto& e : pr->pool) { (void)hipEventDestroy(e.first); (void)hipEventDestroy(e.second); }
    }
    delete pr;
    return CTTS_OK;
}

static size_t packed_bf16_bytes_impl(const ctts_waveglow_config* cfg, int P) {
    Plan p; BfPlan q;
    if (make_plan(cfg, p)) return 0;
    if (p.C % BGEMM_KC != 0 || p.H % BGEMM_KC != 0) { set_error("bf16: channels must be multiples of 32"); return 0; }
    make_bf_plan(p, q, P);
    return q.total * sizeof(bf16_t);
}

static int pack_flow_bf16_impl(const ctts_waveglow_config* cfg, int32_t k, const ctts_waveglow_flow_weights* w,
                               void* packed_bf16, void* stream, int P, int f16 = 0) {
    Plan p; BfPlan q;
    int rc = make_plan(cfg, p); if (rc) return rc;
    CTTS_CHECK_ARG(k >= 0 && k < p.c.n_flows && w && packed_bf16, "pack_flow_bf16: bad argument");
    CTTS_CHECK_ARG(p.C % BGEMM_KC == 0 && p.H % BGEMM_KC == 0, "pack_flow_bf16: channels must be multiples of 32");
    CTTS_CHECK_ARG(!f16 || P == 1, "pack_flow: the split form exists for bf16 only");
    make_bf_plan(p, q, P, f16);
    CTTS_CHECK_ARG(q.nch_in <= BGEMM_MAX_CHUNKS && BF_SKIP_GROUP * q.nch_rs <= BGEMM_MAX_CHUNKS,
                   "pack_flow_bf16: K of %d chunks exceeds the chunk table", q.nch_in);
    hipStream_t s = as_stream(stream);
    bf16_t* bb = static_cast<bf16_t*>(packed_bf16);
    const int C = p.C, H = p.H, ks = p.c.kernel_size;
    CTTS_CHECK_ARG(w->cond_w[0] && w->cond_w[1] && p.K0 % BGEMM_KC == 0, "pack_flow_bf16: cond weights / n_mel*n_group %% 32");
    const int sdim = p.c.speaker_embed_dim;
    bf16_t* c0 = bb + q.cond0_A + (size_t)k * q.nch_c0 * BGEMM_KC * BGEMM_BM;
    bf16_t* c1 = bb + q.cond1_A + (size_t)k * q.nch_c1 * BGEMM_KC * BGEMM_BM;
// ... 163 lines not shown
```

### cookietts_amd/csrc/waveglow_kernels.h

```cpp
#pragma once

#include "common.h"
#include "gemm_f32.h"

namespace ctts {

int launch_fold_weightnorm(const float* v, const float* g, float* w, int out_ch, int fan, hipStream_t s);
int launch_pack_a(float* dst, const float* src, int bm, int MB, int nch_total, int k_off, int ksrc, int epi, int C, int M,
                  long long src_row_off, long long src_row_stride, int src_k_stride, hipStream_t s, int k_group = 1,
                  int k_member = 0);
int launch_pack_bias(float* dst, int bm, int MB, const float* src0, long long off0, const float* src1, long long off1,
                     int epi, int C, int M, hipStream_t s);
bool upsample_mfma_shape(int n_mel, int win, int hop, int G);
int launch_upsample_pack_mfma(const float* W, float* Wp, hipStream_t s);
int launch_upsample_squeeze(const float* mel, const float* W, const float* Wp, const float* bias, float* spect, int batch,
                            int n_mel, int F, int win, int hop, int G, int ld, int pad, hipStream_t s);
int launch_wn_start(const float* audio, const float* Ws, const float* bs, float* x, int batch, int C, int G,
                    int ch_off, int n_half, int L, int ld, int pad, hipStream_t s);
struct CouplingForward {
    float* log_s;
    long long ls_bstride;
    double* part;
    long long part_bstride;
};
constexpr int FWD_SUMSQ_CHUNK = 4096;
int launch_flow_tail(const float* out, float* audio, float* wave, const float* Wend, const float* bend,
                     const float* Winv, int batch, int C, int G, int ch_off, int n_half, int L, int ld, int pad,
                     hipStream_t s, const CouplingForward* fwd = nullptr);
int launch_flow_head_forward(const float* W, const float* wave, float* z, int batch, int G, int ch_off, int n_rem, int L,
                             hipStream_t s);
int launch_sumsq_partials(const float* z, double* part, int batch, long long n_item, int nblk, hipStream_t s);
int launch_sum_partials(const double* part, long long part_bstride, long long part_kstride, int n, double* out, int out_bstride,
                        int nk, int batch, hipStream_t s);

constexpr int FOLD_ROWS = 16;
int launch_fold_in0(const float* in_w, const float* Ws, const float* bs, float* dst, int C, int n_half, int ks, hipStream_t s);
int launch_fold_skend(const float* const* rs_w, const float* const* rs_b, const float* Wend, const float* bend, float* Wf,
                      float* bf, int C, int n_layers, int n_half, hipStream_t s);
int launch_wn_start_ones(const float* audio, float* a16, int batch, int G, int ch_off, int n_half, int L, int ld, int pad,
                         hipStream_t s);
int launch_skip_end(const float* act, long long act_stride, int nl, const float* Wf, float* acc, bool first, bool tail,
                    const float* bf, const float* Winv, float* audio, float* wave, int batch, int C, int G, int ch_off,
                    int n_half, int L, int ld, int pad, hipStream_t s, const CouplingForward* fwd = nullptr);

int launch_winograd_g(const float* in_w, float* dense, int rows, int C, hipStream_t s);
int launch_winograd_transform(const float* x, long long x_bstride, const float* h2, long long h_bstride, float* V, float* Hc,
                              int batch, int C, int H, int d, int L, int Lp, int ld, int pad, int ldp, int ncols, bool cond_rows,
                              bool vec_d2, hipStream_t s);

int launch_winograd_g43(const float* in_w, float* dense, int rows, int C, hipStream_t s);
int launch_winograd_transform_quad(const float* x, long long x_bstride, const float* h2, long long h_bstride, float* V, float* Hc,
                                   int batch, int C, int H, int d, int L, int Lq, int ld, int pad, int ldq, int ncols, bool cond_rows,
                                   hipStream_t s);

}
```

### cookietts_amd/csrc/waveglow_kernels.hip

```cpp
#include "waveglow_kernels.h"
#include "tuning.h"

namespace ctts {

namespace {

__global__ __launch_bounds__(256) void fold_weightnorm_kernel(const float* __restrict__ v,
                                                              const float* __restrict__ g,
                                                              float* __restrict__ w, int fan) {
    __shared__ float red[4];
    const int o = blockIdx.x;
    const float* vr = v + (size_t)o * fan;
    float s = 0.f;
    for (int i = threadIdx.x; i < fan; i += 256) { const float x = vr[i]; s = fmaf(x, x, s); }
#pragma unroll
    for (int off = 32; off > 0; off >>= 1) s += __shfl_xor(s, off);
    if ((threadIdx.x & 63) == 0) red[threadIdx.x >> 6] = s;
    __syncthreads();
    const float tot = red[0] + red[1] + red[2] + red[3];
    const float scale = g[o] / sqrtf(tot);
    float* wr = w + (size_t)o * fan;
    for (int i = threadIdx.x; i < fan; i += 256) wr[i] = vr[i] * scale;
}

// ... 530 lines not shown
    dense[2 * (size_t)n + idx] = (float)(-(w0 - w1 + w2) / 6.0);
    dense[3 * (size_t)n + idx] = (float)(w0 / 24.0 + w1 / 12.0 + w2 / 6.0);
    dense[4 * (size_t)n + idx] = (float)(w0 / 24.0 - w1 / 12.0 + w2 / 6.0);
    dense[5 * (size_t)n + idx] = in_w[(size_t)idx * 3 + 2];
}

template <int MODE>
__global__ __launch_bounds__(256) void winograd_transform_quad_kernel(const float* __restrict__ x, long long x_bstride,
                                                                      const float* __restrict__ h2, long long h_bstride,
                                                                      float* __restrict__ V, float* __restrict__ Hc, int C, int H,
                                                                      int d, int L, int Lq, int ld, int pad, int ldq, int ncols) {
    const int q4 = (blockIdx.x * 256 + threadIdx.x) * 4;
    if (q4 >= ncols) return;
    const int row = blockIdx.y, b = blockIdx.z, B = gridDim.z;
    const bool is_x = row < C;
    const float* src = is_x ? x + (size_t)b * x_bstride + (size_t)row * ld + pad
                            : h2 + (size_t)b * h_bstride + (size_t)(row - C) * ld + pad;
    float tap[6][4];
#pragma unroll
    for (int j = 0; j < 6; ++j)
#pragma unroll
        for (int e = 0; e < 4; ++e) tap[j][e] = 0.f;
    [[maybe_unused]] auto ld4 = [&](int t) { return (t >= 0 && t < L) ? *reinterpret_cast<const float4*>(src + t) : make_float4(0.f, 0.f, 0.f, 0.f); };
    if constexpr (MODE == 1) {
        if (q4 < Lq) {
            const int t0 = (q4 / d) * 4 * d + q4 % d;
#pragma unroll
            for (int j = 0; j < 6; ++j) {
                if (!is_x && (j == 0 || j == 5)) continue;
                const float4 v = ld4(t0 + (j - 1) * d);
                tap[j][0] = v.x; tap[j][1] = v.y; tap[j][2] = v.z; tap[j][3] = v.w;
            }
        }
    } else if constexpr (MODE == 2) {
        if (q4 < Lq) {
            float a[24];
#pragma unroll
            for (int u = 0; u < 6; ++u) {
                const float4 v = ld4(4 * q4 - 4 + 4 * u);
                a[4 * u] = v.x; a[4 * u + 1] = v.y; a[4 * u + 2] = v.z; a[4 * u + 3] = v.w;
            }
            const bool hi = q4 + 2 < Lq;
#pragma unroll
            for (int j = 0; j < 6; ++j) {
                tap[j][0] = a[4 + (j - 1) * 2]; tap[j][1] = a[5 + (j - 1) * 2];
                tap[j][2] = hi ? a[12 + (j - 1) * 2] : 0.f; tap[j][3] = hi ? a[13 + (j - 1) * 2] : 0.f;
            }
        }
    } else {
#pragma unroll
        for (int e = 0; e < 4; ++e) {
            const int q = q4 + e;
            const int t0 = (q / d) * 4 * d + q % d;
#pragma unroll
            for (int j = 0; j < 6; ++j) {
                const int t = t0 + (j - 1) * d;
                tap[j][e] = (q < Lq && t >= 0 && t < L && (is_x || (j >= 1 && j <= 4))) ? src[t] : 0.f;
            }
        }
    }
    if (is_x) {
        const size_t plane = (size_t)B * C * ldq;
        float* o = V + ((size_t)b * C + row) * ldq + q4;
        float v[6][4];
#pragma unroll
        for (int e = 0; e < 4; ++e) {
            const float x0 = tap[0][e], x1 = tap[1][e], x2 = tap[2][e], x3 = tap[3][e], x4 = tap[4][e], x5 = tap[5][e];
            const float s12 = x1 + x2, d12 = x1 - x2, s34 = x3 + x4, d34 = x3 - x4, d13 = x1 - x3, d24 = x2 - x4;
            v[0][e] = 4.f * x0 - 5.f * x2 + x4;
            v[1][e] = s34 - 4.f * s12;
            v[2][e] = 4.f * d12 - d34;
            v[3][e] = -2.f * d13 - d24;
            v[4][e] = 2.f * d13 - d24;
            v[5][e] = 4.f * x1 - 5.f * x3 + x5;
        }
#pragma unroll
        for (int j = 0; j < 6; ++j) *reinterpret_cast<float4*>(o + j * plane) = make_float4(v[j][0], v[j][1], v[j][2], v[j][3]);
    } else {
        const size_t plane = (size_t)B * H * ldq;
        float* o = Hc + ((size_t)b * H + (row - C)) * ldq + q4;
#pragma unroll
        for (int k = 0; k < 4; ++k) *reinterpret_cast<float4*>(o + k * plane) = make_float4(tap[k + 1][0], tap[k + 1][1], tap[k + 1][2], tap[k + 1][3]);
    }
}

template <int H>
__global__ __launch_bounds__(256) void wn_start_ones_kernel(const float* __restrict__ audio, float* __restrict__ a16, int G,
                                                            int ch_off, int L, int ld, int pad) {
    const int col = (blockIdx.x * 256 + threadIdx.x) * 4;
    const int b = blockIdx.z;
    if (col >= ld) return;
    const int n = col - pad;
    const bool in = n >= 0 && n < L;
    float* dst = a16 + (size_t)b * FOLD_ROWS * ld + col;
#pragma unroll
    for (int r = 0; r < FOLD_ROWS; ++r) {
        float4 v = make_float4(0.f, 0.f, 0.f, 0.f);
        if (in && r < H) v = *reinterpret_cast<const float4*>(audio + ((size_t)b * G + ch_off + r) * L + n);
        else if (in && r == H) v = make_float4(1.f, 1.f, 1.f, 1.f);
        *reinterpret_cast<float4*>(dst + (size_t)r * ld) = v;
    }
}

enum { SKEND_ACC = 0, SKEND_TAIL = 1, SKEND_FWD = 2 };
template <int H, int TAIL>
__global__ __launch_bounds__(256) void skip_end_kernel(const float* __restrict__ act, long long act_stride, int nl,
                                                       const float* __restrict__ Wf, float* __restrict__ acc, int first,
                                                       const float* __restrict__ bf, const float* __restrict__ Winv,
                                                       float* __restrict__ audio, float* __restrict__ wave,
                                                       int C, int G, int ch_off, int L, int ld, int pad, CouplingForward fw) {
    constexpr int E = 2 * H;
    constexpr int NG = E <= 4 ? 8 : E <= 8 ? 4 : 2;
    __shared__ __attribute__((aligned(16))) float part[3][E][256];
    __shared__ float sWinv[E * E];
    const int lane = threadIdx.x & 63;
    const int wv = threadIdx.x >> 6;
    const int b = blockIdx.y;
    const int n = blockIdx.x * 256 + lane * 4;
    if (TAIL == SKEND_TAIL && threadIdx.x < E * E) sWinv[threadIdx.x] = Winv[threadIdx.x];
    float4 e[E];
#pragma unroll
    for (int j = 0; j < E; ++j) e[j] = make_float4(0.f, 0.f, 0.f, 0.f);
    const int cq = C / 4;
    const int cbeg = __builtin_amdgcn_readfirstlane(wv * cq);
    for (int l = 0; l < nl; ++l) {
        const float* ob = act + (size_t)l * act_stride + (size_t)b * C * ld + pad + n;
        const float* wl = Wf + (size_t)l * C * E;
        for (int c = cbeg; c < cbeg + cq; c += NG) {
            float4 v[NG];
#pragma unroll
            for (int k = 0; k < NG; ++k) v[k] = *reinterpret_cast<const float4*>(ob + (size_t)(c + k) * ld);
#pragma unroll
            for (int k = 0; k < NG; ++k)
#pragma unroll
                for (int j = 0; j < E; ++j) {
                    const float w = wl[(c + k) * E + j];
                    e[j].x = fmaf(w, v[k].x, e[j].x); e[j].y = fmaf(w, v[k].y, e[j].y);
                    e[j].z = fmaf(w, v[k].z, e[j].z); e[j].w = fmaf(w, v[k].w, e[j].w);
                }
        }
    }
    if (wv > 0) {
#pragma unroll
        for (int j = 0; j < E; ++j) *reinterpret_cast<float4*>(&part[wv - 1][j][lane * 4]) = e[j];
    }
    __syncthreads();
    if (wv != 0 || (TAIL != SKEND_FWD && n >= L)) return;
    float* ab = acc + (size_t)b * E * ld + pad + n;
#pragma unroll
    for (int j = 0; j < E; ++j) {
#pragma unroll
        for (int q = 0; q < 3; ++q) {
            const float4 pv = *reinterpret_cast<const float4*>(&part[q][j][lane * 4]);
            e[j].x += pv.x; e[j].y += pv.y; e[j].z += pv.z; e[j].w += pv.w;
        }
        if (!first) {
            const float4 pv = *reinterpret_cast<const float4*>(ab + (size_t)j * ld);
            e[j].x += pv.x; e[j].y += pv.y; e[j].z += pv.z; e[j].w += pv.w;
        }
    }
    if constexpr (TAIL == SKEND_ACC) {
#pragma unroll
        for (int j = 0; j < E; ++j) *reinterpret_cast<float4*>(ab + (size_t)j * ld) = e[j];
    } else {
#pragma unroll
        for (int j = 0; j < E; ++j) {
// ... 125 lines not shown
    }
#undef CTTS_TAIL_CASE
    CTTS_CHECK_LAUNCH("flow_tail");
    return CTTS_OK;
}

int launch_fold_in0(const float* in_w, const float* Ws, const float* bs, float* dst, int C, int n_half, int ks, hipStream_t s) {
    CTTS_CHECK_ARG(n_half >= 1 && n_half < FOLD_ROWS, "fold_in0: n_half=%d", n_half);
    const int n = 2 * C * FOLD_ROWS * ks;
    hipLaunchKernelGGL(fold_in0_kernel, dim3((n + 255) / 256), dim3(256), 0, s, in_w, Ws, bs, dst, C, n_half, ks, 2 * C);
    CTTS_CHECK_LAUNCH("fold_in0");
    return CTTS_OK;
}

int launch_fold_skend(const float* const* rs_w, const float* const* rs_b, const float* Wend, const float* bend, float* Wf,
                      float* bf, int C, int n_layers, int n_half, hipStream_t s) {
    const int E = 2 * n_half;
    CTTS_CHECK_ARG(n_layers >= 1 && n_layers <= 12 && E <= 64, "fold_skend: n_layers=%d n_half=%d", n_layers, n_half);
    SkipBiasPtrs sb{};
    for (int i = 0; i < n_layers; ++i) {
        CTTS_CHECK_ARG(rs_w[i] && rs_b[i], "fold_skend: NULL layer %d weights", i);
        const int row_off = i < n_layers - 1 ? C : 0;
        sb.p[i] = rs_b[i];
        sb.row_off[i] = row_off;
        hipLaunchKernelGGL(fold_skend_w_kernel, dim3((C * E + 255) / 256), dim3(256), 0, s, Wend, rs_w[i], Wf + (size_t)i * C * E,
                           C, E, row_off);
    }
    hipLaunchKernelGGL(fold_skend_b_kernel, dim3(1), dim3(64), 0, s, Wend, bend, sb, n_layers, bf, C, E);
    CTTS_CHECK_LAUNCH("fold_skend");
    return CTTS_OK;
}

int launch_winograd_g(const float* in_w, float* dense, int rows, int C, hipStream_t s) {
    const int n = rows * C;
    hipLaunchKernelGGL(winograd_g_kernel, dim3((n + 255) / 256), dim3(256), 0, s, in_w, dense, n);
    CTTS_CHECK_LAUNCH("winograd_g");
    return CTTS_OK;
}

int launch_winograd_transform(const float* x, long long x_bstride, const float* h2, long long h_bstride, float* V, float* Hc,
                              int batch, int C, int H, int d, int L, int Lp, int ld, int pad, int ldp, int ncols, bool cond_rows,
                              bool vec_d2, hipStream_t s) {
    CTTS_CHECK_ARG(d >= 1 && Lp % d == 0 && (long long)Lp * 2 >= L && Lp <= ncols && ncols <= ldp && ncols % 4 == 0 && ldp % 4 == 0 &&
                       ld % 4 == 0 && pad % 4 == 0 && pad + L <= ld,
                   "winograd_transform: d=%d L=%d Lp=%d ncols=%d ldp=%d ld=%d pad=%d", d, L, Lp, ncols, ldp, ld, pad);
    dim3 grid((ncols / 4 + 255) / 256, cond_rows ? C + H : C, batch);
    if (d % 4 == 0 && L % 4 == 0)
        hipLaunchKernelGGL(winograd_transform_kernel<1>, grid, dim3(256), 0, s, x, x_bstride, h2, h_bstride, V, Hc, C, H, d, L, Lp,
                           ld, pad, ldp, ncols);
    else if (d == 2 && L % 4 == 0 && vec_d2)
        hipLaunchKernelGGL(winograd_transform_kernel<2>, grid, dim3(256), 0, s, x, x_bstride, h2, h_bstride, V, Hc, C, H, d, L, Lp,
                           ld, pad, ldp, ncols);
    else
        hipLaunchKernelGGL(winograd_transform_kernel<0>, grid, dim3(256), 0, s, x, x_bstride, h2, h_bstride, V, Hc, C, H, d, L, Lp,
                           ld, pad, ldp, ncols);
    CTTS_CHECK_LAUNCH("winograd_transform");
    return CTTS_OK;
}

int launch_winograd_g43(const float* in_w, float* dense, int rows, int C, hipStream_t s) {
    const int n = rows * C;
    hipLaunchKernelGGL(winograd_g43_kernel, dim3((n + 255) / 256), dim3(256), 0, s, in_w, dense, n);
    CTTS_CHECK_LAUNCH("winograd_g43");
    return CTTS_OK;
}

int launch_winograd_transform_quad(const float* x, long long x_bstride, const float* h2, long long h_bstride, float* V, float* Hc,
                                   int batch, int C, int H, int d, int L, int Lq, int ld, int pad, int ldq, int ncols, bool cond_rows,
                                   hipStream_t s) {
    CTTS_CHECK_ARG(d >= 1 && Lq % d == 0 && (long long)Lq * 4 >= L && Lq <= ncols && ncols <= ldq && ncols % 4 == 0 && ldq % 4 == 0 &&
                       ld % 4 == 0 && pad % 4 == 0 && pad + L <= ld && (!cond_rows || Hc != nullptr),
                   "winograd_transform_quad: d=%d L=%d Lq=%d ncols=%d ldq=%d ld=%d pad=%d", d, L, Lq, ncols, ldq, ld, pad);
    dim3 grid((ncols / 4 + 255) / 256, cond_rows ? C + H : C, batch);
    if (d % 4 == 0 && L % 4 == 0)
        hipLaunchKernelGGL(winograd_transform_quad_kernel<1>, grid, dim3(256), 0, s, x, x_bstride, h2, h_bstride, V, Hc, C, H, d, L, Lq,
                           ld, pad, ldq, ncols);
    else if (d == 2 && L % 4 == 0)
        hipLaunchKernelGGL(winograd_transform_quad_kernel<2>, grid, dim3(256), 0, s, x, x_bstride, h2, h_bstride, V, Hc, C, H, d, L, Lq,
                           ld, pad, ldq, ncols);
    else
        hipLaunchKernelGGL(winograd_transform_quad_kernel<0>, grid, dim3(256), 0, s, x, x_bstride, h2, h_bstride, V, Hc, C, H, d, L, Lq,
                           ld, pad, ldq, ncols);
    CTTS_CHECK_LAUNCH("winograd_transform_quad");
    return CTTS_OK;
}

int launch_wn_start_ones(const float* audio, float* a16, int batch, int G, int ch_off, int n_half, int L, int ld, int pad,
                         hipStream_t s) {
    CTTS_CHECK_ARG(L % 4 == 0 && ld % 4 == 0 && pad % 4 == 0, "wn_start_ones: L=%d ld=%d pad=%d", L, ld, pad);
    dim3 grid((ld / 4 + 255) / 256, 1, batch);
#define CTTS_ONES_CASE(H)                                                                                     \
    case H:                                                                                                   \
        hipLaunchKernelGGL(wn_start_ones_kernel<H>, grid, dim3(256), 0, s, audio, a16, G, ch_off, L, ld, pad); \
        break;
    switch (n_half) {
        CTTS_ONES_CASE(1) CTTS_ONES_CASE(2) CTTS_ONES_CASE(3) CTTS_ONES_CASE(4)
        CTTS_ONES_CASE(5) CTTS_ONES_CASE(6) CTTS_ONES_CASE(7) CTTS_ONES_CASE(8)
        default:
            set_error("wn_start_ones: n_half=%d unsupported (1..8)", n_half);
            return CTTS_E_ARG;
    }
#undef CTTS_ONES_CASE
    CTTS_CHECK_LAUNCH("wn_start_ones");
    return CTTS_OK;
}

int launch_skip_end(const float* act, long long act_stride, int nl, const float* Wf, float* acc, bool first, bool tail,
                    const float* bf, const float* Winv, float* audio, float* wave, int batch, int C, int G, int ch_off,
                    int n_half, int L, int ld, int pad, hipStream_t s, const CouplingForward* fwd) {
    CTTS_CHECK_ARG(fwd == nullptr || (tail && fwd->part != nullptr && wave == nullptr), "skip_end: forward direction on the tail pass only");
    const CouplingForward fw = fwd ? *fwd : CouplingForward{};
    CTTS_CHECK_ARG(L % 4 == 0 && C % 32 == 0 && ld % 4 == 0 && pad % 4 == 0 && nl >= 1, "skip_end: L=%d C=%d nl=%d", L, C, nl);
    CTTS_CHECK_ARG(acc != nullptr || (first && tail), "skip_end: a group after the first needs the accumulator");
    CTTS_CHECK_ARG(!tail || wave == nullptr || (ch_off == 0 && 2 * n_half == G && G % 4 == 0),
                   "skip_end: un-squeeze needs the full group (ch_off=%d n_half=%d G=%d)", ch_off, n_half, G);
    dim3 grid((L + 255) / 256, batch);
    const int fi = first ? 1 : 0;
#define CTTS_SKEND_CASE(H)                                                                                                \
    case H:                                                                                                               \
        if (fwd)                                                                                                          \
            hipLaunchKernelGGL((skip_end_kernel<H, SKEND_FWD>), grid, dim3(256), 0, s, act, act_stride, nl, Wf, acc, fi, bf, Winv, \
                               audio, wave, C, G, ch_off, L, ld, pad, fw);                                                \
        else if (tail)                                                                                                    \
            hipLaunchKernelGGL((skip_end_kernel<H, SKEND_TAIL>), grid, dim3(256), 0, s, act, act_stride, nl, Wf, acc, fi, bf, Winv, \
                               audio, wave, C, G, ch_off, L, ld, pad, fw);                                                \
        else                                                                                                              \
            hipLaunchKernelGGL((skip_end_kernel<H, SKEND_ACC>), grid, dim3(256), 0, s, act, act_stride, nl, Wf, acc, fi, bf, Winv, \
                               audio, wave, C, G, ch_off, L, ld, pad, fw);                                                \
        break;
    switch (n_half) {
        CTTS_SKEND_CASE(1) CTTS_SKEND_CASE(2) CTTS_SKEND_CASE(3) CTTS_SKEND_CASE(4)
        CTTS_SKEND_CASE(5) CTTS_SKEND_CASE(6) CTTS_SKEND_CASE(7) CTTS_SKEND_CASE(8)
        default:
            set_error("skip_end: n_half=%d unsupported (1..8)", n_half);
            return CTTS_E_ARG;
    }
#undef CTTS_SKEND_CASE
    CTTS_CHECK_LAUNCH("skip_end");
    return CTTS_OK;
}

int launch_flow_head_forward(const float* W, const float* wave, float* z, int batch, int G, int ch_off, int n_rem, int L,
                             hipStream_t s) {
    CTTS_CHECK_ARG(L % 4 == 0 && n_rem >= 2 && n_rem % 2 == 0 && ch_off >= 0 && ch_off + n_rem == G,
                   "flow_head_forward: L=%d n_rem=%d ch_off=%d G=%d", L, n_rem, ch_off, G);
    CTTS_CHECK_ARG(wave == nullptr || (ch_off == 0 && G % 4 == 0), "flow_head_forward: the squeeze needs the full group (ch_off=%d G=%d)",
                   ch_off, G);
    dim3 grid((L / 4 + 255) / 256, batch);
#define CTTS_HEAD_LAUNCH(EE, SQ) \
    hipLaunchKernelGGL((flow_head_forward_kernel<EE, SQ>), grid, dim3(256), 0, s, W, wave, z, G, ch_off, L)
#define CTTS_HEAD_CASE(EE)             \
    case EE:                           \
        CTTS_HEAD_LAUNCH(EE, false);   \
        break;
#define CTTS_HEAD_CASE_SQ(EE)                                                       \
    case EE:                                                                        \
        if (wave) CTTS_HEAD_LAUNCH(EE, true); else CTTS_HEAD_LAUNCH(EE, false);     \
        break;
    switch (n_rem) {
        CTTS_HEAD_CASE(2) CTTS_HEAD_CASE_SQ(4) CTTS_HEAD_CASE(6) CTTS_HEAD_CASE_SQ(8)
        CTTS_HEAD_CASE(10) CTTS_HEAD_CASE_SQ(12) CTTS_HEAD_CASE(14) CTTS_HEAD_CASE_SQ(16)
        default:
            set_error("flow_head_forward: n_rem=%d unsupported (2..16, even)", n_rem);
            return CTTS_E_ARG;
    }
#undef CTTS_HEAD_CASE_SQ
// ... 24 lines not shown
```

### cookietts_amd/csrc/wn_winograd_layer.h

```cpp
#pragma once

#include "common.h"
#include "gemm_f32.h"

namespace ctts {

constexpr int WNWG_MAX_CHUNKS = 320;
constexpr int WNWG_F23 = 0, WNWG_F43 = 1;

struct WnWinogradLayerArgs {
    const float *A_T2, *A_T3, *A_e, *A_o, *bias;
    const float *A_T4, *A_T5;
    const float* V; long long vplane;
    const float* Hc; long long hplane;
    const float* h2; long long h_bstride;
    float* act; long long act_bstride;
    int C, H, batch;
    int ldp, Lp, ntiles;
    int d, L, ld, pad;
    int in_place;
    int form;
    int kt, kt_total, b0, col0;
};

bool wn_winograd_layer_supported(int C, int H);
bool wn_winograd_layer_f43_supported(int C, int H);
int launch_wn_winograd_layer(const WnWinogradLayerArgs& a, hipStream_t stream);
int last_wn_winograd_f43_width();

}
```

### cookietts_amd/csrc/wn_winograd_layer.hip

```cpp
#include "wn_winograd_layer.h"
#include "tuning.h"

namespace ctts {

typedef float wg_f32x16 __attribute__((ext_vector_type(16)));
typedef unsigned wg_u32x4 __attribute__((ext_vector_type(4)));

namespace {

__device__ __forceinline__ float wg_sigmoid(float u) {
    return __builtin_amdgcn_rcpf(1.0f + __builtin_amdgcn_exp2f(u * -1.4426950408889634f));
}
__device__ __forceinline__ float wg_tanh(float u) {
    return 1.0f - 2.0f * __builtin_amdgcn_rcpf(1.0f + __builtin_amdgcn_exp2f(u * 2.8853900817779268f));
}

}

template <int NT, int F43, int KD, int TP>
__global__ __launch_bounds__(256, (F43 && NT == 2) ? 1 : 2) void wn_winograd_layer_f32_kernel(const WnWinogradLayerArgs a) {
    static_assert(KD == 1 || (KD == 2 && F43 && TP), "two chunks per stage: the F(4,3) form (its phases are whole stages, see the launcher)");
    constexpr int NI = F43 ? 4 : 2;
    constexpr int BN = 64 * NT;
    constexpr int A_ST = GEMM_KC * 128;
    constexpr int CST = A_ST + GEMM_KC * BN;
    constexpr int STG = KD * CST;
    constexpr int NP = 2 + NT;
    constexpr int TAB = 3 * STG;
    constexpr int BIAS = TAB + 4 * WNWG_MAX_CHUNKS;
    constexpr int UPR = BN / 4;
    constexpr int RPP = 64 / UPR;
    __shared__ __attribute__((aligned(16))) float lds[BIAS + 128];

    const int t = threadIdx.x;
    const int lane = t & 63;
    const int wave = __builtin_amdgcn_readfirstlane(t >> 6);
    const int wm = wave >> 1, wn = wave & 1;
    const int l31 = lane & 31, lhi = lane >> 5;

    const int ncb = a.C >> 6;
    const int jx = blockIdx.x >> 3;
    const int cb = jx % ncb;
    const int gt = (jx / ncb) * 8 + (blockIdx.x & 7);
    if (gt >= a.kt_total) return;
    const int b = a.b0 + gt / a.kt;
    const int n0 = a.col0 + (gt % a.kt) * BN;

    const int n1 = a.C / GEMM_KC, n2 = (a.C + a.H) / GEMM_KC, nh = a.H / GEMM_KC;
    const int c_e = NI * n1;
    int ps[NI + 1];
    ps[0] = c_e;
#pragma unroll
    for (int k = 0; k < NI; ++k) ps[k + 1] = ps[k] + (k == 0 || k == NI - 1 ? n2 : nh);
    const int nch = ps[NI];

    const int mb_t = (64 * cb) >> 8, loc_t = (64 * cb) & 255;
    const int mb_s = (a.C + 64 * cb) >> 8, loc_s = (a.C + 64 * cb) & 255;
    {
        uint4* tab = reinterpret_cast<uint4*>(lds + TAB);
        for (int c = t; c < nch; c += 256) {
            const float *ap, *bp;
            if (c < c_e) {
                const int ph = F43 ? c / n1 : (int)(c >= n1), loc = c - ph * n1;
                ap = (ph == 0 ? a.A_T2 : ph == 1 ? a.A_T3 : ph == 2 ? a.A_T4 : a.A_T5) + ((size_t)mb_t * n1 + loc) * (GEMM_KC * 256) + loc_t;
                bp = a.V + (1 + ph) * a.vplane + ((size_t)b * a.C + (size_t)loc * GEMM_KC) * a.ldp + n0;
            } else {
                int ph = 0;
#pragma unroll
                for (int k = 1; k < NI; ++k) ph += c >= ps[k];
                const bool last = ph == NI - 1;
                const int loc = c - ps[ph] + (ph == 0 || last ? 0 : n1);
                ap = (last ? a.A_o : a.A_e) + ((size_t)(cb >> 1) * n2 + loc) * (GEMM_KC * 256) + (cb & 1) * 128;
                if (loc < n1) bp = a.V + (last ? NI + 1 : 0) * a.vplane + ((size_t)b * a.C + (size_t)loc * GEMM_KC) * a.ldp + n0;
                else if (a.in_place) bp = a.h2 + (size_t)b * a.h_bstride + (size_t)(loc - n1) * GEMM_KC * a.ld;
                else bp = a.Hc + ph * a.hplane + ((size_t)b * a.H + (size_t)(loc - n1) * GEMM_KC) * a.ldp + n0;
            }
            const unsigned long long ua = reinterpret_cast<unsigned long long>(ap), ub = reinterpret_cast<unsigned long long>(bp);
            tab[c] = make_uint4((unsigned)ua, (unsigned)(ua >> 32), (unsigned)ub, (unsigned)(ub >> 32));
        }
        if (t < 128) lds[BIAS + t] = a.bias[cb * 128 + t];
    }

    unsigned offa_g[2], offa_s[2], offb[NT], offb_m[NI][NT];
    {
        const int col = (lane & 31) * 4;
        const long long delta = ((long long)(mb_s - mb_t) * n1) * (GEMM_KC * 256) + (loc_s - loc_t);
#pragma unroll
        for (int j = 0; j < 2; ++j) {
            const int krow = 2 * (wave + 4 * j) + (lane >> 5);
            offa_g[j] = (unsigned)((krow * 256 + col) * 4);
            offa_s[j] = (unsigned)((krow * 256 + (col < 64 ? (long long)col : col - 64 + delta)) * 4);
        }
        const int bcol = (lane % UPR) * 4;
#pragma unroll
        for (int j = 0; j < NT; ++j) {
            const int krow = (wave + 4 * j) * RPP + lane / UPR;
            offb[j] = (unsigned)(((size_t)krow * a.ldp + bcol) * 4);
#pragma unroll
            for (int k = 0; k < NI; ++k) offb_m[k][j] = 0;
            if (a.in_place) {
                const int q = n0 + bcol;
                const int te = (q / a.d) * (NI * a.d) + q % a.d;
                const int lim = (a.ld - a.pad - 4) & ~3;
#pragma unroll
                for (int k = 0; k < NI; ++k) offb_m[k][j] = (unsigned)(((size_t)krow * a.ld + a.pad + min(te + k * a.d, lim)) * 4);
            }
        }
    }
    int m_lo[NI];
#pragma unroll
    for (int k = 0; k < NI; ++k) m_lo[k] = a.in_place ? ps[k] + (k == 0 || k == NI - 1 ? n1 : 0) : 0x7fffffff;

    wg_f32x16 X[NI][2][NT];
#pragma unroll
    for (int k = 0; k < NI; ++k)
#pragma unroll
        for (int i = 0; i < 2; ++i)
#pragma unroll
            for (int j = 0; j < NT; ++j)
#pragma unroll
                for (int r = 0; r < 16; ++r) X[k][i][j][r] = 0.0f;
    __syncthreads();

    typedef __attribute__((address_space(3))) float* lds_fptr;
    typedef const __attribute__((address_space(1))) float* gfloat_ptr;
    typedef const __attribute__((address_space(1))) char* gbyte_ptr;
    const wg_u32x4* ctab = reinterpret_cast<const wg_u32x4*>(lds + TAB);
    wg_u32x4 tn_[KD];
    const unsigned tab_lds = (unsigned)reinterpret_cast<uintptr_t>((lds_fptr)(lds + TAB));
#define WNWG_TAB_ISSUE(c)                                                                                   \
    _Pragma("unroll") for (int j = 0; j < KD; ++j) asm volatile("ds_read_b128 %0, %1" : "=v"(tn_[j]) : "v"(tab_lds + 16u * (unsigned)((c) + j)));
#define WNWG_TAB_WAIT()                                                                                     \
    do {                                                                                                    \
        if constexpr (KD == 2) asm volatile("s_waitcnt lgkmcnt(0)" : "+v"(tn_[0]), "+v"(tn_[KD - 1]) : : "memory"); \
        else asm volatile("s_waitcnt lgkmcnt(0)" : "+v"(tn_[0]) : : "memory");                              \
    } while (0)
#define WNWG_ADDR(buf, c)                                                                                   \
    lds_fptr la_ = (lds_fptr)(lds + (buf) * STG + wave * 256);                                              \
    wg_u32x4 e_[KD];                                                                                        \
    _Pragma("unroll") for (int j = 0; j < KD; ++j) {                                                        \
        if constexpr (TP) e_[j] = tn_[j];                                                                   \
        else e_[j] = ctab[(c) + j];                                                                         \
    }                                                                                                       \
    const bool as_ = (c) < c_e;                                       \
    bool mk_[NI];                                                     \
    _Pragma("unroll") for (int k = 0; k < NI; ++k) mk_[k] = (c) >= m_lo[k] && (c) < ps[k + 1];
#define WNWG_BASES()                                                                                        \
// ... 82 lines not shown
    _Pragma("unroll") for (int nt = 0; nt < NT; ++nt) fb[r][nt] = (Bp)[((r) >> 3) * CST + (2 * ((r) & 7) + lhi) * BN + nt * 32];
#define WNWG_MM(Y, r)                                                                                       \
    _Pragma("unroll") for (int mt = 0; mt < 2; ++mt)                                                        \
        _Pragma("unroll") for (int nt = 0; nt < NT; ++nt)                                                   \
            Y[mt][nt] = __builtin_amdgcn_mfma_f32_32x32x2f32(fa[r][mt], fb[r][nt], Y[mt][nt], 0, 0, 0);
#define WNWG_R2(Y, r)                                                                                       \
    __builtin_amdgcn_sched_barrier(0);                                                                      \
    WNWG_RD((r) + 1, As, Bs)                                                                                \
    WNWG_MM(Y, r)                                                                                           \
    WNWG_PIECE(r);
#define WNWG_CHUNK2(Y)                                                                                      \
    {                                                                                                       \
        const float* As = lds + cur * STG + wm * 32 + l31;                                                  \
        const float* Bs = lds + cur * STG + A_ST + wn * (32 * NT) + l31;                                    \
        const int nx = cur == 2 ? 0 : cur + 1;                                                              \
        const float* An = lds + nx * STG + wm * 32 + l31;                                                   \
        const float* Bn = lds + nx * STG + A_ST + wn * (32 * NT) + l31;                                     \
        const int nb = cur >= 1 ? cur - 1 : 2;                      \
        const int cn = ch + 2 * KD < nch ? ch + 2 * KD : nch - KD;                                          \
        WNWG_ADDR(nb, cn)                                                                                   \
        __builtin_amdgcn_sched_barrier(0);                                                                  \
        WNWG_BASES()                                                                                        \
        WNWG_R2(Y, 0) WNWG_R2(Y, 1) WNWG_R2(Y, 2) WNWG_R2(Y, 3) WNWG_R2(Y, 4) WNWG_R2(Y, 5) WNWG_R2(Y, 6) WNWG_R2(Y, 7)   \
        WNWG_R2(Y, 8) WNWG_R2(Y, 9)                                                                         \
        WNWG_TAB_ISSUE(ch + 3 * KD < nch ? ch + 3 * KD : nch - KD)                                          \
        WNWG_R2(Y, 10) WNWG_R2(Y, 11) WNWG_R2(Y, 12) WNWG_R2(Y, 13) WNWG_R2(Y, 14)                          \
        __builtin_amdgcn_sched_barrier(0);                                                                  \
        WNWG_TAB_WAIT();                                                \
        WNWG_WAIT();                                         \
        __builtin_amdgcn_s_barrier();                                                                       \
        __builtin_amdgcn_sched_barrier(0);                                                                  \
        WNWG_RD(0, An, Bn)                                                                                  \
        WNWG_MM(Y, 15)                                                                                      \
        __builtin_amdgcn_sched_barrier(0);                                                                  \
        cur = nx;                                                                                           \
    }
#define WNWG_CHUNK(Y)                                                                                       \
    if constexpr (KD == 1) WNWG_CHUNK1(Y) else WNWG_CHUNK2(Y)
    if constexpr (KD == 2) {
        const float* As = lds + wm * 32 + l31;
        const float* Bs = lds + A_ST + wn * (32 * NT) + l31;
        WNWG_RD(0, As, Bs)
    }

    float* dst = a.act + (size_t)b * a.act_bstride + (size_t)(cb * 64 + wm * 32) * a.ld + a.pad;
    const float* bias = lds + BIAS + wm * 32;
#define WNWG_GATE(Y, par)                                                                                   \
    _Pragma("unroll") for (int nt = 0; nt < NT; ++nt) {                                                     \
        const int n = n0 + wn * (32 * NT) + nt * 32 + l31;                                                  \
        const int ns = (n / a.d) * (NI * a.d) + n % a.d + (par) * a.d;                                      \
        if (n < a.Lp && ns < a.L) {                                                                         \
            _Pragma("unroll") for (int r = 0; r < 16; ++r) {                                                \
                const int row = (r & 3) + 8 * (r >> 2) + 4 * lhi;                                           \
                const float u0 = Y[0][nt][r] + bias[row];                                                   \
                const float u1 = Y[1][nt][r] + bias[64 + row];                                              \
                dst[(size_t)row * a.ld + ns] = wg_tanh(u0) * wg_sigmoid(u1);                                \
            }                                                                                               \
        }                                                                                                   \
    }

#define WNWG_RUN(k, end) for (; ch < (end); ch += KD) WNWG_CHUNK(X[k])
#define WNWG_DRAIN()                                                                                        \
    asm volatile("s_waitcnt vmcnt(0)" ::: "memory");          \
    __builtin_amdgcn_s_barrier();
    int ch = 0;
    if constexpr (!F43) {
        WNWG_RUN(0, n1)
        WNWG_RUN(1, c_e)
#pragma unroll
        for (int i = 0; i < 2; ++i)
#pragma unroll
            for (int j = 0; j < NT; ++j)
#pragma unroll
                for (int r = 0; r < 16; ++r) {
                    const float s = X[0][i][j][r], dd = X[1][i][j][r];
                    X[0][i][j][r] = s + dd;
                    X[1][i][j][r] = s - dd;
                }
        WNWG_RUN(0, ps[1])
        WNWG_GATE(X[0], 0)
        WNWG_RUN(1, nch)
        WNWG_DRAIN()
        WNWG_GATE(X[1], 1)
    } else {
        WNWG_RUN(0, n1)
        WNWG_RUN(1, 2 * n1)
        WNWG_RUN(2, 3 * n1)
        WNWG_RUN(3, c_e)
#pragma unroll
        for (int i = 0; i < 2; ++i)
#pragma unroll
            for (int j = 0; j < NT; ++j)
#pragma unroll
                for (int r = 0; r < 16; ++r) {
                    if constexpr (NT == 2)
                        if (r == 0) asm volatile("" : "+a"(X[0][i][j]), "+a"(X[1][i][j]), "+a"(X[2][i][j]), "+a"(X[3][i][j]));
                    const float p1 = X[0][i][j][r], p2 = X[1][i][j][r], p3 = X[2][i][j][r], p4 = X[3][i][j][r];
                    const float sa = p1 + p2, sb = p1 - p2, sc = p3 + p4, se = p3 - p4;
                    X[0][i][j][r] = sa + sc;
                    X[1][i][j][r] = sb + 2.0f * se;
                    X[2][i][j][r] = sa + 4.0f * sc;
                    X[3][i][j][r] = sb + 8.0f * se;
                    if constexpr (NT == 2)
                        if (r == 15) asm volatile("" : "+a"(X[0][i][j]), "+a"(X[1][i][j]), "+a"(X[2][i][j]), "+a"(X[3][i][j]));
                }
#pragma unroll
        for (int k = 0; k < NI; ++k)
#pragma unroll
            for (int i = 0; i < 2; ++i) {
                if constexpr (NT == 2) { asm volatile("" : "+a"(X[k][i][0])); asm volatile("" : "+a"(X[k][i][1])); }
                else asm volatile("" : "+v"(X[k][i][0]));
            }
        WNWG_RUN(0, ps[1])
        WNWG_GATE(X[0], 0)
        WNWG_RUN(1, ps[2])
        WNWG_GATE(X[1], 1)
        WNWG_RUN(2, ps[3])
        WNWG_GATE(X[2], 2)
        WNWG_RUN(3, nch)
        WNWG_DRAIN()
        WNWG_GATE(X[3], 3)
    }
#undef WNWG_DRAIN
#undef WNWG_RUN
#undef WNWG_GATE
#undef WNWG_CHUNK
#undef WNWG_CHUNK2
#undef WNWG_R2
#undef WNWG_MM
#undef WNWG_RD
#undef WNWG_CHUNK1
#undef WNWG_REGION
#undef WNWG_MFMA
#undef WNWG_READ_FRAGS
#undef WNWG_WAIT
#undef WNWG_PIECE
#undef WNWG_BASES
#undef WNWG_TAB_WAIT
#undef WNWG_TAB_ISSUE
#undef WNWG_ADDR
}

bool wn_winograd_layer_supported(int C, int H) {
    return C >= 128 && C % 128 == 0 && H > 0 && H % GEMM_KC == 0 && 2 * (C / GEMM_KC) + 2 * ((C + H) / GEMM_KC) <= WNWG_MAX_CHUNKS;
}

bool wn_winograd_layer_f43_supported(int C, int H) {
    return wn_winograd_layer_supported(C, H) && 4 * (C / GEMM_KC) + 2 * ((C + H) / GEMM_KC) + 2 * (H / GEMM_KC) <= WNWG_MAX_CHUNKS;
}

namespace {
thread_local int t_last_f43_width = 0;

template <int NT, int F43, int KD, int TP>
int launch_wnwg_shape(WnWinogradLayerArgs a, int kt, long long kt_total, hipStream_t stream) {
    a.kt = kt;
    a.kt_total = (int)kt_total;
    const long long blocks = 8ll * (a.C / 64) * ((kt_total + 7) / 8);
    CTTS_CHECK_ARG(blocks > 0 && blocks < (1ll << 31) && kt_total < (1ll << 31), "wn_winograd_layer: grid %lld", blocks);
    hipLaunchKernelGGL((wn_winograd_layer_f32_kernel<NT, F43, KD, TP>), dim3((unsigned)blocks), dim3(256), 0, stream, a);
    CTTS_CHECK_LAUNCH("wn_winograd_layer");
    return CTTS_OK;
}

}

int last_wn_winograd_f43_width() { return t_last_f43_width; }

int launch_wn_winograd_layer(const WnWinogradLayerArgs& a_in, hipStream_t stream) {
    WnWinogradLayerArgs a = a_in;
    CTTS_CHECK_ARG(wn_winograd_layer_supported(a.C, a.H), "wn_winograd_layer: C=%d H=%d", a.C, a.H);
    CTTS_CHECK_ARG(a.A_T2 && a.A_T3 && a.A_e && a.A_o && a.bias && a.V && a.act && a.batch >= 1, "wn_winograd_layer: operand not set");
    const bool f43 = a.form == WNWG_F43;
    const int tw = f43 ? 64 : 128;
    CTTS_CHECK_ARG(a.form == WNWG_F23 || (f43 && wn_winograd_layer_f43_supported(a.C, a.H) && a.A_T4 && a.A_T5), "wn_winograd_layer: form %d", a.form);
    CTTS_CHECK_ARG(a.d >= 1 && a.L >= 1 && a.Lp >= 1 && a.ntiles >= 1 && a.Lp <= a.ntiles * tw && a.ntiles * tw <= a.ldp && a.ldp % 4 == 0 &&
                       a.ld % 4 == 0 && a.pad >= 0 && a.pad % 4 == 0 && a.L + a.pad <= a.ld,
                   "wn_winograd_layer: geometry d=%d L=%d Lp=%d ntiles=%d ldp=%d ld=%d pad=%d", a.d, a.L, a.Lp, a.ntiles, a.ldp, a.ld, a.pad);
    CTTS_CHECK_ARG(a.in_place ? (a.h2 && a.d % 4 == 0 && a.ld - a.pad >= 4 && a.h_bstride % 4 == 0 && reinterpret_cast<uintptr_t>(a.h2) % 16 == 0)
                              : a.Hc != nullptr,
                   "wn_winograd_layer: cond rows (in_place=%d d=%d)", a.in_place, a.d);
    a.b0 = 0;
    a.col0 = 0;
    const Tuning tn = tuning();
    if (f43) {
        const bool kd2 = a.H % (2 * GEMM_KC) == 0;
        if (tn.f32_no_small && kd2) {
            const int wt = (a.ntiles + 1) / 2;
            CTTS_CHECK_ARG((long long)wt * 128 <= a.ldp, "wn_winograd_layer: %d tiles of 128 quad columns beyond ldp=%d", wt, a.ldp);
            t_last_f43_width = 128;
            return launch_wnwg_shape<2, 1, 2, 1>(a, wt, (long long)wt * a.batch, stream);
        }
        t_last_f43_width = 64;
        if (tn.f32_force_small || !kd2) return launch_wnwg_shape<1, 1, 1, 0>(a, a.ntiles, (long long)a.ntiles * a.batch, stream);
        return launch_wnwg_shape<1, 1, 2, 1>(a, a.ntiles, (long long)a.ntiles * a.batch, stream);
    }
    const int ncb = a.C / 64;
    const long long slots = 2ll * wf_row_cus();
    const int kt_narrow = (a.Lp + 63) / 64;
    long long tiles = (long long)a.ntiles * a.batch;
    if (!tn.f32_no_small && (tn.f32_force_small || ncb * tiles < 2 * slots)) return launch_wnwg_shape<1, 0, 1, 0>(a, kt_narrow, (long long)kt_narrow * a.batch, stream);
    if (!tn.f32_no_round_split && !tn.f32_no_small) {
        const long long rounds = ncb * tiles / slots;
        const long long rem_tiles = (ncb * tiles - rounds * slots + ncb - 1) / ncb;
        if (rounds >= 2 && rem_tiles > 0 && rem_tiles * ncb <= slots * 3 / 10 && rem_tiles < a.ntiles &&
            (long long)(a.ntiles - rem_tiles) * 128 < a.Lp) {
            WnWinogradLayerArgs r = a;
            r.b0 = a.batch - 1;
            r.col0 = (int)(a.ntiles - rem_tiles) * 128;
            const int kt = (a.Lp - r.col0 + 63) / 64;
            if (int rc = launch_wnwg_shape<1, 0, 1, 0>(r, kt, kt, stream)) return rc;
            tiles -= rem_tiles;
        }
    }
    return launch_wnwg_shape<2, 0, 1, 0>(a, a.ntiles, tiles, stream);
}

}
```

### include/cookietts_hip.h

```cpp
#ifndef COOKIETTS_HIP_H
#define COOKIETTS_HIP_H

#include <stddef.h>
#include <stdint.h>

#ifdef __cplusplus
extern "C" {
#endif

#define CTTS_OK 0
#define CTTS_E_ARG (-1)
#define CTTS_E_LAUNCH (-2)
#define CTTS_E_WORKSPACE (-3)
#define CTTS_E_ABORT (-4)

#define CTTS_ABI_VERSION 7

#define CTTS_GEMM_DEFAULT 0
#define CTTS_GEMM_F32 1
#define CTTS_GEMM_BF16X3 2
#define CTTS_GEMM_BF16X6 3
#define CTTS_WG_OPT_COMPOSED_COND 1
#define CTTS_N_SPEAKERS 512

// ... 555 lines not shown
    double diagonality_weighting, max_focus_weighting, min_focus_weighting, avg_focus_weighting;
    double target_score, absolutely_required_score;
    int32_t max_attempts, absolute_maximum_tries;
    int32_t n_texts, per_text;
    int32_t n_mel, t_cap, enc_cap;
} ctts_retry_config;

typedef struct ctts_retry_status {
    int32_t done;
    int32_t n_passes;
    double min_best_score;
    int32_t min_tries;
    int32_t n_without_winner;
    int32_t max_best_length;
    int32_t max_best_T;
} ctts_retry_status;

size_t ctts_retry_state_bytes(const ctts_retry_config* cfg);
#define CTTS_RETRY_SECTIONS 14
int ctts_retry_state_layout(const ctts_retry_config* cfg, size_t* offsets);
int ctts_retry_reset(const ctts_retry_config* cfg, void* state, void* stream);
int ctts_retry_update_f32(const ctts_retry_config* cfg, const float* mel, const float* gate, const float* alignments,
                          const double* metrics, const int32_t* output_lengths, const int32_t* text_lengths, int32_t T,
                          int32_t enc, double* detail, void* state, void* stream);
int ctts_retry_vocoder_batch_f32(const ctts_retry_config* cfg, const void* state, float* mel_out, int32_t t_out,
                                 float pad_value, void* stream);
int ctts_pcm16_concat(const void* audio, int32_t is_half, const int32_t* frames, int32_t batch, int64_t ld, int32_t hop,
                      int32_t silence_samples, int16_t* pcm, int64_t pcm_capacity, int64_t* offsets, void* stream);

#define CTTS_TACO_LOSS_COLUMNS 27
#define CTTS_TACO_LOSS_TERMS 13
typedef struct {
    double gate_positive_weight;
    double sigma;
    double weights[9];
} ctts_taco_loss_params;
size_t ctts_taco_loss_workspace_bytes(int32_t batch, int32_t n_mel, int32_t T, int32_t enc);
int ctts_taco_loss_f32(const ctts_taco_loss_params* params, const float* pred_mel, const float* pred_mel_postnet,
                       const float* gt_mel, const float* gate_logits, const float* gate_target, const float* alignments,
                       const float* sylps_mu, const float* sylps_logvar, const float* pred_sylps, const float* gt_sylps,
                       const int32_t* mel_lengths, const int32_t* text_lengths, const float* pres_prev_state, int32_t batch,
                       int32_t n_mel, int32_t T, int32_t enc, double* table, double* terms, void* workspace,
                       size_t workspace_bytes, void* stream);
int ctts_taco_loss_finalize_f32(const ctts_taco_loss_params* params, const double* metric_gt, const double* metric_pred,
                                const float* sylps_mu, const float* sylps_logvar, const float* pred_sylps,
                                const float* gt_sylps, const int32_t* mel_lengths, const int32_t* text_lengths,
                                const float* pres_prev_state, int32_t batch, int32_t n_mel, int32_t T, int32_t enc,
                                double* table, double* terms, const void* workspace, size_t workspace_bytes, void* stream);

#define CTTS_MEL_ERROR_MAX_WINDOWS 8
#define CTTS_MEL_ERROR_COLUMNS 5
#define CTTS_MEL_ERROR_TERMS (2 + CTTS_MEL_ERROR_MAX_WINDOWS)
#define CTTS_MEL_ERROR_TACOTRON 0
#define CTTS_MEL_ERROR_NV 1
#define CTTS_MEL_ERROR_SANITIZE 1
typedef struct ctts_mel_error_config {
    int32_t n_windows;
    int32_t filter_lengths[CTTS_MEL_ERROR_MAX_WINDOWS];
    int32_t hop_length;
    int32_t n_mel_channels;
    int32_t framing;
    float clamp_val;
    float mag_eps;
} ctts_mel_error_config;
size_t ctts_mel_error_packed_bytes(const ctts_mel_error_config* cfg);
int ctts_mel_error_pack(const ctts_mel_error_config* cfg, int32_t window, const float* forward_basis, const float* mel_basis,
                        void* packed, void* stream);
size_t ctts_mel_error_workspace_bytes(const ctts_mel_error_config* cfg, int32_t batch, int32_t T_pred_max, int32_t T_gt_max);
int ctts_mel_error_f32(const ctts_mel_error_config* cfg, const void* packed, const float* pred, const int32_t* pred_lengths,
                       const float* gt, const int32_t* gt_lengths, const float* gt_mel, int32_t flags, int32_t batch,
                       int32_t T_pred, int32_t T_gt, int32_t mel_frames, double* table, float* mae_map, float* pred_map,
                       float* gt_map, int32_t map_frames, void* workspace, size_t workspace_bytes, void* stream);

int ctts_mel_dtw_f32(const float* pred, const float* target, const int32_t* lengths, float* out, int32_t* choice, float* l1,
                     int32_t batch, int32_t channels, int32_t frames, int32_t scale_factor, int32_t range, void* stream);
int ctts_mel_dtw_generic_f32(const float* pred, const float* target, const int32_t* lengths, float* out, int32_t* choice, float* l1,
                             int32_t batch, int32_t channels, int32_t frames, int32_t scale_factor, int32_t range, void* stream);

int ctts_last_gemm_loop(void);
int ctts_last_winograd_f43_width(void);

int ctts_tuning_reload(void);
int ctts_tuning_flags(void);

#define CTTS_PROF_WN_IN 0
#define CTTS_PROF_WN_RS 1
#define CTTS_PROF_WN_SKIP 2
#define CTTS_PROF_WN_IN0F 3
#define CTTS_PROF_WN_SKEND 4
#define CTTS_PROF_WN_RES_F 5
#define CTTS_PROF_N 6
int ctts_profile_create(void** handle);
int ctts_profile_bind(void* handle);
int ctts_profile_collect(void* handle, int32_t which, int64_t* launches, double* total_ms);
int ctts_profile_destroy(void* handle);

#ifdef __cplusplus
}
#endif
#endif
```

Before: 4.068 million samples/s.

## Add Winograd F(6,3) path for in-place WN dilated conv layers

```diff
diff --git a/cookietts_amd/_lib.py b/cookietts_amd/_lib.py
--- a/cookietts_amd/_lib.py
+++ b/cookietts_amd/_lib.py
@@ -359,6 +359,7 @@
     "ctts_last_winograd_f43_width": (C.c_int, []),
     "ctts_tuning_reload": (C.c_int, []),
     "ctts_tuning_flags": (C.c_int, []),
+    "ctts_tuning_flags_ext": (C.c_int, []),
     "ctts_profile_create": (C.c_int, [C.POINTER(C.c_void_p)]),
     "ctts_profile_bind": (C.c_int, [C.c_void_p]),
     "ctts_profile_collect": (C.c_int, [C.c_void_p, C.c_int32, C.POINTER(C.c_int64), C.POINTER(C.c_double)]),
@@ -429,7 +430,7 @@
                "CTTS_F32_WINOGRAD_NO_F43": 22,
                "CTTS_TACO_POLL_DELAY": 23, "CTTS_TACO_VALU": 24, "CTTS_UP_NO_MFMA": 25, "CTTS_F32_NO_WN_FOLD": 26, "CTTS_TACO_BG_NO_PIPE": 27,
                "CTTS_F32_NO_WINOGRAD": 28, "CTTS_F32_WINOGRAD_MIN": 29, "CTTS_F32_WINOGRAD_PLAIN": 30}
-TUNING_BITS_EXT = {"CTTS_WF_FWD_ROWWISE": 31}
+TUNING_BITS_EXT = {"CTTS_WF_FWD_ROWWISE": 31, "CTTS_F32_WINOGRAD_F63_MIN": 32, "CTTS_F32_WINOGRAD_NO_F63": 33}
 
 
 def tuning_reload():
@@ -438,6 +439,8 @@
 
 def tuning_active(name):
     bit = TUNING_BITS[name] if name in TUNING_BITS else TUNING_BITS_EXT[name]
+    if bit >= 32:
+        return bool(lib().ctts_tuning_flags_ext() >> (bit - 32) & 1)
     return bool(lib().ctts_tuning_flags() >> bit & 1)
 
 
diff --git a/cookietts_amd/csrc/gemm_f32.hip b/cookietts_amd/csrc/gemm_f32.hip
--- a/cookietts_amd/csrc/gemm_f32.hip
+++ b/cookietts_amd/csrc/gemm_f32.hip
@@ -777,6 +777,8 @@
     g_tune.f32_winograd_no_fused = on("CTTS_F32_WINOGRAD_NO_FUSED");
     g_tune.f32_winograd_f43_min = num("CTTS_F32_WINOGRAD_F43_MIN", -1);
     g_tune.f32_winograd_no_f43 = on("CTTS_F32_WINOGRAD_NO_F43");
+    g_tune.f32_winograd_f63_min = num("CTTS_F32_WINOGRAD_F63_MIN", -1);
+    g_tune.f32_winograd_no_f63 = on("CTTS_F32_WINOGRAD_NO_F63");
     g_tune.f32_cond_chain = on("CTTS_F32_COND_CHAIN");
     g_tune_loaded = true;
 }
diff --git a/cookietts_amd/csrc/tuning.h b/cookietts_amd/csrc/tuning.h
--- a/cookietts_amd/csrc/tuning.h
+++ b/cookietts_amd/csrc/tuning.h
@@ -28,6 +28,8 @@
     bool f32_winograd_plain;
     int f32_winograd_fused_min;
     int f32_winograd_f43_min;
+    int f32_winograd_f63_min;
+    bool f32_winograd_no_f63;
     bool f32_winograd_no_f43;
     bool f32_winograd_no_fused;
     bool f32_cond_chain;
diff --git a/cookietts_amd/csrc/waveglow_api.hip b/cookietts_amd/csrc/waveglow_api.hip
--- a/cookietts_amd/csrc/waveglow_api.hip
+++ b/cookietts_amd/csrc/waveglow_api.hip
@@ -48,6 +48,7 @@
         std::vector<size_t> wg_T2_A, wg_T3_A, wg_e_A, wg_o_A;
         size_t wg_dense;
         std::vector<size_t> wq_U_A[4], wq_e_A, wq_o_A;
+        std::vector<size_t> wh_U_A[6], wh_e_A, wh_o_A;
     };
     std::vector<Flow> fl;
     size_t total;
@@ -59,6 +60,8 @@
     int rs_rows(int layer) const { return layer < c.n_layers - 1 ? 2 * C : C; }
     int rs_mb(int layer) const { return (rs_rows(layer) + GEMM_BM - 1) / GEMM_BM; }
 };
+
+bool f63_layer(int layer) { return (1 << layer) % 4 == 0; }
 
 int make_plan(const ctts_waveglow_config* cfg, Plan& p, int options = 0) {
     CTTS_CHECK_ARG(cfg != nullptr, "config is NULL");
@@ -144,7 +147,14 @@
             f.wq_e_A.push_back(take((size_t)p.mb_in * (p.nch_rs + p.nch1h) * A_TILE));
             f.wq_o_A.push_back(take((size_t)p.mb_in * (p.nch_rs + p.nch1h) * A_TILE));
         }
-        f.wg_dense = take((size_t)(f43 ? 6 : 3) * 2 * p.C * p.C);
+        const bool f63 = wn_winograd_layer_f63_supported(p.C, p.H);
+        for (int i = 0; f63 && i < c.n_layers; ++i) {
+            const bool on = f63_layer(i);
+            for (auto& u : f.wh_U_A) u.push_back(on ? take((size_t)p.mb_in * p.nch_rs * A_TILE) : 0);
+            f.wh_e_A.push_back(on ? take((size_t)p.mb_in * (p.nch_rs + p.nch1h) * A_TILE) : 0);
+            f.wh_o_A.push_back(on ? take((size_t)p.mb_in * (p.nch_rs + p.nch1h) * A_TILE) : 0);
+        }
+        f.wg_dense = take((size_t)(f63 ? 8 : f43 ? 6 : 3) * 2 * p.C * p.C);
     }
     p.ccP = c.hop_length / c.n_group;
     p.ccJ = c.win_length / c.hop_length;
@@ -195,11 +205,23 @@
     for (int i = 0; i < p.c.n_layers; ++i) nt = std::max(nt, quad_geom(g, i).ntiles);
     return round_up(nt * 64, 128);
 }
-enum class InForm { Direct, WinogradSeparate, WinogradPaired, WinogradLayer, WinogradLayerF43 };
+PairGeom hex_geom(const Geom& g, int layer) {
+    const int d = 1 << layer;
+    const int Lh = (g.L + 6 * d - 1) / (6 * d) * d;
+    return {d, Lh, (Lh + 63) / 64};
+}
+int hex_ld(const Plan& p, const Geom& g) {
+    int nt = 0;
+    for (int i = 0; i < p.c.n_layers; ++i) nt = std::max(nt, hex_geom(g, i).ntiles);
+    return nt * 64;
+}
+enum class InForm { Direct, WinogradSeparate, WinogradPaired, WinogradLayer, WinogradLayerF43, WinogradLayerF63 };
+bool quad_space(InForm in) { return in == InForm::WinogradLayerF43 || in == InForm::WinogradLayerF63; }
 
 constexpr long long WINOGRAD_MIN_COLS = 28800;
 constexpr long long WINOGRAD_FUSED_MIN_COLS = 28800;
 constexpr long long WINOGRAD_F43_MIN_COLS = 28800;
+constexpr long long WINOGRAD_F63_MIN_COLS = 28800;
 
 InForm in_form(const Plan& p, const Geom& g, const Tuning& t) {
     auto long_enough = [&](int knob, long long cols) { return (long long)g.L >= (knob >= 0 ? knob : cols); };
@@ -211,7 +233,9 @@
         return InForm::WinogradPaired;
     if (t.f32_winograd_no_f43 || !wn_winograd_layer_f43_supported(p.C, p.H) || !long_enough(t.f32_winograd_f43_min, WINOGRAD_F43_MIN_COLS))
         return InForm::WinogradLayer;
-    return InForm::WinogradLayerF43;
+    if (t.f32_winograd_no_f63 || !wn_winograd_layer_f63_supported(p.C, p.H) || !long_enough(t.f32_winograd_f63_min, WINOGRAD_F63_MIN_COLS))
+        return InForm::WinogradLayerF43;
+    return InForm::WinogradLayerF63;
 }
 
 bool cond_composed(const Plan& p, int frames, const Tuning& t) {
@@ -232,7 +256,7 @@
     float* a16;
     float* skend;
     float *wgV, *wgT, *wgH;
-    int ldp, ldq;
+    int ldp, ldq, ldh;
     size_t total;
 };
 
@@ -253,11 +277,12 @@
     w.a16 = take(B * FOLD_ROWS * g.ld);
     w.skend = take(B * p.c.n_group * g.ld);
     w.wgV = w.wgT = w.wgH = nullptr;
-    w.ldp = w.ldq = 0;
+    w.ldp = w.ldq = w.ldh = 0;
     if (in != InForm::Direct) {
         w.ldp = pair_ld(p, g);
-        w.ldq = in == InForm::WinogradLayerF43 ? quad_ld(p, g) : 0;
-        w.wgV = take(std::max((size_t)4 * w.ldp, (size_t)6 * w.ldq) * B * p.C);
+        w.ldq = quad_space(in) ? quad_ld(p, g) : 0;
+        w.ldh = in == InForm::WinogradLayerF63 ? hex_ld(p, g) : 0;
+        w.wgV = take(std::max({(size_t)4 * w.ldp, (size_t)6 * w.ldq, (size_t)8 * w.ldh}) * B * p.C);
         w.wgT = take((size_t)2 * B * 2 * p.C * w.ldp);
         w.wgH = take(std::max((size_t)2 * w.ldp, (size_t)4 * w.ldq) * B * p.H);
     }
@@ -420,6 +445,7 @@
     float* act(int i) const { return stack == StackForm::PerLayer ? w.act : w.act_all + (size_t)(i % Plan::F32_SKIP_GROUP) * act_stride(); }
     bool group_ends(int i) const { return i == p.c.n_layers - 1 || (i + 1) % Plan::F32_SKIP_GROUP == 0; }
     bool in_place(int i) const { return in != InForm::WinogradSeparate && (1 << i) % 4 == 0; }
+    bool hex(int i) const { return in == InForm::WinogradLayerF63 && f63_layer(i); }
     size_t plane(int rows) const { return (size_t)batch * rows * w.ldp; }
 
     GemmArgs header() const {
@@ -546,11 +572,16 @@
     }
     WnWinogradLayerArgs wg_layer(int k, int i) const {
         const auto& f = p.fl[k];
-        const bool f43 = in == InForm::WinogradLayerF43;
-        const PairGeom sg = f43 ? quad_geom(g, i) : pair_geom(g, i);
-        const int ldw = f43 ? w.ldq : w.ldp;
+        const bool f43 = quad_space(in) && !hex(i);
+        const PairGeom sg = hex(i) ? hex_geom(g, i) : f43 ? quad_geom(g, i) : pair_geom(g, i);
+        const int ldw = hex(i) ? w.ldh : f43 ? w.ldq : w.ldp;
         WnWinogradLayerArgs a{};
-        if (f43) {
+        if (hex(i)) {
+            a.form = WNWG_F63;
+            a.A_T2 = blob + f.wh_U_A[0][i]; a.A_T3 = blob + f.wh_U_A[1][i]; a.A_T4 = blob + f.wh_U_A[2][i]; a.A_T5 = blob + f.wh_U_A[3][i];
+            a.A_T6 = blob + f.wh_U_A[4][i]; a.A_T7 = blob + f.wh_U_A[5][i];
+            a.A_e = blob + f.wh_e_A[i]; a.A_o = blob + f.wh_o_A[i];
+        } else if (f43) {
             a.form = WNWG_F43;
             a.A_T2 = blob + f.wq_U_A[0][i]; a.A_T3 = blob + f.wq_U_A[1][i]; a.A_T4 = blob + f.wq_U_A[2][i]; a.A_T5 = blob + f.wq_U_A[3][i];
             a.A_e = blob + f.wq_e_A[i]; a.A_o = blob + f.wq_o_A[i];
@@ -574,7 +605,11 @@
         return launch_gemm_f32(epi, a, s);
     }
     int wg_transform(int k, int i) const {
-        if (in == InForm::WinogradLayerF43) {
+        if (hex(i)) {
+            const PairGeom hg = hex_geom(g, i);
+            return launch_winograd_transform_hex(w.x, cstride, w.wgV, batch, p.C, hg.d, g.L, hg.Lp, g.ld, g.pad, w.ldh, hg.ntiles * 64, s);
+        }
+        if (quad_space(in)) {
             const PairGeom qg = quad_geom(g, i);
             const int ncols = t.f32_no_small ? round_up(qg.ntiles * 64, 128) : qg.ntiles * 64;
             return launch_winograd_transform_quad(w.x, cstride, h(k), hstride, w.wgV, w.wgH, batch, p.C, p.H, qg.d, g.L, qg.Lp, g.ld, g.pad,
@@ -594,6 +629,7 @@
             return launch_gemm_f32(GEMM_EPI_GATE, in_gemm(k, i), s);
         case InForm::WinogradLayer:
         case InForm::WinogradLayerF43:
+        case InForm::WinogradLayerF63:
             return launch_wn_winograd_layer(wg_layer(k, i), s);
         case InForm::WinogradSeparate:
         case InForm::WinogradPaired:
@@ -1136,6 +1172,16 @@
         if ((rc = pack_gate(f.wq_e_A[i], dense, C, 1, i))) return rc;
         if ((rc = pack_gate(f.wq_o_A[i], dense + 5 * dn, C, 1, i))) return rc;
     }
+    for (int i = 0; i < (f.wh_e_A.empty() ? 0 : p.c.n_layers); ++i) {
+        if (!f63_layer(i)) continue;
+        float* dense = blob + f.wg_dense;
+        const size_t dn = (size_t)2 * C * C;
+        if ((rc = launch_winograd_g63(w->in_w[i], dense, 2 * C, C, s))) return rc;
+        for (int j = 0; j < 6; ++j)
+            if ((rc = launch_pack_a(blob + f.wh_U_A[j][i], dense + (1 + j) * dn, GEMM_BM, p.mb_in, p.nch_rs, 0, C, GEMM_EPI_SPLIT, C, 2 * C, 0, C, 1, s))) return rc;
+        if ((rc = pack_gate(f.wh_e_A[i], dense, C, 1, i))) return rc;
+        if ((rc = pack_gate(f.wh_o_A[i], dense + 7 * dn, C, 1, i))) return rc;
+    }
     if ((rc = launch_fold_in0(w->in_w[0], w->start_w, w->start_b, blob + f.in0f_w, C, d.n_half, ks, s))) return rc;
     for (int t = 0; t < ks; ++t)
         if ((rc = launch_pack_a(blob + f.in0f_A, blob + f.in0f_w + t, GEMM_BM, p.mb_in, p.nch_in0f, 0, FOLD_ROWS, GEMM_EPI_GATE, C,
@@ -1355,6 +1401,10 @@
 int ctts_last_gemm_loop(void) { return last_gemm_loop(); }
 int ctts_last_winograd_f43_width(void) { return last_wn_winograd_f43_width(); }
 int ctts_tuning_reload(void) { reload_tuning(); return CTTS_OK; }
+int ctts_tuning_flags_ext(void) {
+    const Tuning t = tuning();
+    return (t.f32_winograd_f63_min >= 0 ? 1 : 0) | (t.f32_winograd_no_f63 ? 2 : 0);
+}
 int ctts_tuning_flags(void) {
     const Tuning t = tuning();
     return (t.f32_no_glds ? 1 : 0) | (t.no_xcd_pair ? 2 : 0) | (t.bf16_no_wide ? 8 : 0) | (t.bf16_no_pp ? 16 : 0) |
diff --git a/cookietts_amd/csrc/waveglow_kernels.h b/cookietts_amd/csrc/waveglow_kernels.h
--- a/cookietts_amd/csrc/waveglow_kernels.h
+++ b/cookietts_amd/csrc/waveglow_kernels.h
@@ -53,4 +53,8 @@
                                    int batch, int C, int H, int d, int L, int Lq, int ld, int pad, int ldq, int ncols, bool cond_rows,
                                    hipStream_t s);
 
+int launch_winograd_g63(const float* in_w, float* dense, int rows, int C, hipStream_t s);
+int launch_winograd_transform_hex(const float* x, long long x_bstride, float* V, int batch, int C, int d, int L, int Lh, int ld, int pad,
+                                  int ldh, int ncols, hipStream_t s);
+
 }
diff --git a/cookietts_amd/csrc/waveglow_kernels.hip b/cookietts_amd/csrc/waveglow_kernels.hip
--- a/cookietts_amd/csrc/waveglow_kernels.hip
+++ b/cookietts_amd/csrc/waveglow_kernels.hip
@@ -636,6 +636,75 @@
 #pragma unroll
         for (int k = 0; k < 4; ++k) *reinterpret_cast<float4*>(o + k * plane) = make_float4(tap[k + 1][0], tap[k + 1][1], tap[k + 1][2], tap[k + 1][3]);
     }
+}
+
+
+__global__ __launch_bounds__(256) void winograd_g63_kernel(const float* __restrict__ in_w, float* __restrict__ dense, int n) {
+    const int idx = blockIdx.x * 256 + threadIdx.x;
+    if (idx >= n) return;
+    const double w0 = in_w[(size_t)idx * 3], w1 = in_w[(size_t)idx * 3 + 1], w2 = in_w[(size_t)idx * 3 + 2];
+    dense[idx] = in_w[(size_t)idx * 3];
+    dense[(size_t)n + idx] = (float)(-2.0 * (w0 + w1 + w2) / 9.0);
+    dense[2 * (size_t)n + idx] = (float)(-2.0 * (w0 - w1 + w2) / 9.0);
+    dense[3 * (size_t)n + idx] = (float)(w0 / 90.0 + w1 / 45.0 + 2.0 * w2 / 45.0);
+    dense[4 * (size_t)n + idx] = (float)(w0 / 90.0 - w1 / 45.0 + 2.0 * w2 / 45.0);
+    dense[5 * (size_t)n + idx] = (float)(32.0 * w0 / 45.0 + 16.0 * w1 / 45.0 + 8.0 * w2 / 45.0);
+    dense[6 * (size_t)n + idx] = (float)(32.0 * w0 / 45.0 - 16.0 * w1 / 45.0 + 8.0 * w2 / 45.0);
+    dense[7 * (size_t)n + idx] = in_w[(size_t)idx * 3 + 2];
+}
+
+template <int MODE>
+__global__ __launch_bounds__(256) void winograd_transform_hex_kernel(const float* __restrict__ x, long long x_bstride, float* __restrict__ V,
+                                                                     int C, int d, int L, int Lh, int ld, int pad, int ldh, int ncols) {
+    const int q4 = (blockIdx.x * 256 + threadIdx.x) * 4;
+    if (q4 >= ncols) return;
+    const int row = blockIdx.y, b = blockIdx.z, B = gridDim.z;
+    const float* src = x + (size_t)b * x_bstride + (size_t)row * ld + pad;
+    float tap[8][4];
+#pragma unroll
+    for (int j = 0; j < 8; ++j)
+#pragma unroll
+        for (int e = 0; e < 4; ++e) tap[j][e] = 0.f;
+    if constexpr (MODE == 1) {
+        if (q4 < Lh) {
+            const int t0 = (q4 / d) * 6 * d + q4 % d;
+#pragma unroll
+            for (int j = 0; j < 8; ++j) {
+                const int t = t0 + (j - 1) * d;
+                if (t < 0 || t >= L) continue;
+                const float4 v = *reinterpret_cast<const float4*>(src + t);
+                tap[j][0] = v.x; tap[j][1] = v.y; tap[j][2] = v.z; tap[j][3] = v.w;
+            }
+        }
+    } else {
+#pragma unroll
+        for (int e = 0; e < 4; ++e) {
+            const int q = q4 + e;
+            const int t0 = (q / d) * 6 * d + q % d;
+#pragma unroll
+            for (int j = 0; j < 8; ++j) {
+                const int t = t0 + (j - 1) * d;
+                tap[j][e] = (q < Lh && t >= 0 && t < L) ? src[t] : 0.f;
+            }
+        }
+    }
+    const size_t plane = (size_t)B * C * ldh;
+    float* o = V + ((size_t)b * C + row) * ldh + q4;
+    float v[8][4];
+#pragma unroll
+    for (int e = 0; e < 4; ++e) {
+        const float x0 = tap[0][e], x1 = tap[1][e], x2 = tap[2][e], x3 = tap[3][e], x4 = tap[4][e], x5 = tap[5][e], x6 = tap[6][e], x7 = tap[7][e];
+        const float e1 = (x2 + x6) - 4.25f * x4, o1 = (x1 + x5) - 4.25f * x3;
+        const float e2 = (0.25f * x2 + x6) - 1.25f * x4, o2 = (0.5f * x1 + 2.f * x5) - 2.5f * x3;
+        const float e3 = (4.f * x2 + x6) - 5.f * x4, o3 = (2.f * x1 + 0.5f * x5) - 2.5f * x3;
+        v[0][e] = (x0 - x6) + 5.25f * (x4 - x2);
+        v[1][e] = e1 + o1; v[2][e] = e1 - o1;
+        v[3][e] = e2 + o2; v[4][e] = e2 - o2;
+        v[5][e] = e3 + o3; v[6][e] = e3 - o3;
+        v[7][e] = (x7 - x1) + 5.25f * (x3 - x5);
+    }
+#pragma unroll
+    for (int j = 0; j < 8; ++j) *reinterpret_cast<float4*>(o + j * plane) = make_float4(v[j][0], v[j][1], v[j][2], v[j][3]);
 }
 
 template <int H>
@@ -927,6 +996,27 @@
         hipLaunchKernelGGL(winograd_transform_quad_kernel<0>, grid, dim3(256), 0, s, x, x_bstride, h2, h_bstride, V, Hc, C, H, d, L, Lq,
                            ld, pad, ldq, ncols);
     CTTS_CHECK_LAUNCH("winograd_transform_quad");
+    return CTTS_OK;
+}
+
+int launch_winograd_g63(const float* in_w, float* dense, int rows, int C, hipStream_t s) {
+    const int n = rows * C;
+    hipLaunchKernelGGL(winograd_g63_kernel, dim3((n + 255) / 256), dim3(256), 0, s, in_w, dense, n);
+    CTTS_CHECK_LAUNCH("winograd_g63");
+    return CTTS_OK;
+}
+
+int launch_winograd_transform_hex(const float* x, long long x_bstride, float* V, int batch, int C, int d, int L, int Lh, int ld, int pad,
+                                  int ldh, int ncols, hipStream_t s) {
+    CTTS_CHECK_ARG(d >= 1 && Lh % d == 0 && (long long)Lh * 6 >= L && Lh <= ncols && ncols <= ldh && ncols % 4 == 0 && ldh % 4 == 0 &&
+                       ld % 4 == 0 && pad % 4 == 0 && pad + L <= ld,
+                   "winograd_transform_hex: d=%d L=%d Lh=%d ncols=%d ldh=%d ld=%d pad=%d", d, L, Lh, ncols, ldh, ld, pad);
+    dim3 grid((ncols / 4 + 255) / 256, C, batch);
+    if (d % 4 == 0 && L % 4 == 0)
+        hipLaunchKernelGGL(winograd_transform_hex_kernel<1>, grid, dim3(256), 0, s, x, x_bstride, V, C, d, L, Lh, ld, pad, ldh, ncols);
+    else
+        hipLaunchKernelGGL(winograd_transform_hex_kernel<0>, grid, dim3(256), 0, s, x, x_bstride, V, C, d, L, Lh, ld, pad, ldh, ncols);
+    CTTS_CHECK_LAUNCH("winograd_transform_hex");
     return CTTS_OK;
 }
 
diff --git a/cookietts_amd/csrc/wn_winograd_layer.h b/cookietts_amd/csrc/wn_winograd_layer.h
--- a/cookietts_amd/csrc/wn_winograd_layer.h
+++ b/cookietts_amd/csrc/wn_winograd_layer.h
@@ -5,12 +5,13 @@
 
 namespace ctts {
 
-constexpr int WNWG_MAX_CHUNKS = 320;
-constexpr int WNWG_F23 = 0, WNWG_F43 = 1;
+constexpr int WNWG_MAX_CHUNKS = 352;
+constexpr int WNWG_F23 = 0, WNWG_F43 = 1, WNWG_F63 = 2;
 
 struct WnWinogradLayerArgs {
     const float *A_T2, *A_T3, *A_e, *A_o, *bias;
     const float *A_T4, *A_T5;
+    const float *A_T6, *A_T7;
     const float* V; long long vplane;
     const float* Hc; long long hplane;
     const float* h2; long long h_bstride;
@@ -25,6 +26,7 @@
 
 bool wn_winograd_layer_supported(int C, int H);
 bool wn_winograd_layer_f43_supported(int C, int H);
+bool wn_winograd_layer_f63_supported(int C, int H);
 int launch_wn_winograd_layer(const WnWinogradLayerArgs& a, hipStream_t stream);
 int last_wn_winograd_f43_width();
 
diff --git a/cookietts_amd/csrc/wn_winograd_layer.hip b/cookietts_amd/csrc/wn_winograd_layer.hip
--- a/cookietts_amd/csrc/wn_winograd_layer.hip
+++ b/cookietts_amd/csrc/wn_winograd_layer.hip
@@ -20,7 +20,8 @@
 template <int NT, int F43, int KD, int TP>
 __global__ __launch_bounds__(256, (F43 && NT == 2) ? 1 : 2) void wn_winograd_layer_f32_kernel(const WnWinogradLayerArgs a) {
     static_assert(KD == 1 || (KD == 2 && F43 && TP), "two chunks per stage: the F(4,3) form (its phases are whole stages, see the launcher)");
-    constexpr int NI = F43 ? 4 : 2;
+    static_assert(F43 <= 1 || (NT == 1 && KD == 2), "the F(6,3) form: 64 hex columns, two chunks per stage");
+    constexpr int NI = 2 + 2 * F43;
     constexpr int BN = 64 * NT;
     constexpr int A_ST = GEMM_KC * 128;
     constexpr int CST = A_ST + GEMM_KC * BN;
@@ -62,7 +63,8 @@
             const float *ap, *bp;
             if (c < c_e) {
                 const int ph = F43 ? c / n1 : (int)(c >= n1), loc = c - ph * n1;
-                ap = (ph == 0 ? a.A_T2 : ph == 1 ? a.A_T3 : ph == 2 ? a.A_T4 : a.A_T5) + ((size_t)mb_t * n1 + loc) * (GEMM_KC * 256) + loc_t;
+                ap = (ph == 0 ? a.A_T2 : ph == 1 ? a.A_T3 : ph == 2 ? a.A_T4 : ph == 3 ? a.A_T5 : ph == 4 ? a.A_T6 : a.A_T7) +
+                     ((size_t)mb_t * n1 + loc) * (GEMM_KC * 256) + loc_t;
                 bp = a.V + (1 + ph) * a.vplane + ((size_t)b * a.C + (size_t)loc * GEMM_KC) * a.ldp + n0;
             } else {
                 int ph = 0;
@@ -311,7 +313,7 @@
         WNWG_RUN(1, nch)
         WNWG_DRAIN()
         WNWG_GATE(X[1], 1)
-    } else {
+    } else if constexpr (F43 == 1) {
         WNWG_RUN(0, n1)
         WNWG_RUN(1, 2 * n1)
         WNWG_RUN(2, 3 * n1)
@@ -349,6 +351,40 @@
         WNWG_RUN(3, nch)
         WNWG_DRAIN()
         WNWG_GATE(X[3], 3)
+    } else {
+        WNWG_RUN(0, n1)
+        WNWG_RUN(1, 2 * n1)
+        WNWG_RUN(2, 3 * n1)
+        WNWG_RUN(3, 4 * n1)
+        WNWG_RUN(4, 5 * n1)
+        WNWG_RUN(5, c_e)
+#pragma unroll
+        for (int i = 0; i < 2; ++i) {
+            asm volatile("" : "+v"(X[0][i][0]), "+v"(X[1][i][0]), "+v"(X[2][i][0]), "+v"(X[3][i][0]), "+v"(X[4][i][0]), "+v"(X[5][i][0]));
+#pragma unroll
+            for (int r = 0; r < 16; ++r) {
+                const float p1 = X[0][i][0][r], p2 = X[1][i][0][r], p3 = X[2][i][0][r], p4 = X[3][i][0][r], p5 = X[4][i][0][r], p6 = X[5][i][0][r];
+                const float sa = p1 + p2, sb = p1 - p2, sc = p3 + p4, se = p3 - p4, sf = p5 + p6, sg = p5 - p6;
+                float y0 = (sa + sc) + sf, y1 = (sb + 2.0f * se) + 0.5f * sg, y2 = (sa + 4.0f * sc) + 0.25f * sf;
+                float y3 = (sb + 8.0f * se) + 0.125f * sg, y4 = (sa + 16.0f * sc) + 0.0625f * sf, y5 = (sb + 32.0f * se) + 0.03125f * sg;
+                asm volatile("" : "+v"(y0), "+v"(y1), "+v"(y2), "+v"(y3), "+v"(y4), "+v"(y5));
+                X[0][i][0][r] = y0; X[1][i][0][r] = y1; X[2][i][0][r] = y2; X[3][i][0][r] = y3; X[4][i][0][r] = y4; X[5][i][0][r] = y5;
+            }
+            asm volatile("" : "+v"(X[0][i][0]), "+v"(X[1][i][0]), "+v"(X[2][i][0]), "+v"(X[3][i][0]), "+v"(X[4][i][0]), "+v"(X[5][i][0]));
+        }
+        WNWG_RUN(0, ps[1])
+        WNWG_GATE(X[0], 0)
+        WNWG_RUN(1, ps[2])
+        WNWG_GATE(X[1], 1)
+        WNWG_RUN(2, ps[3])
+        WNWG_GATE(X[2], 2)
+        WNWG_RUN(3, ps[4])
+        WNWG_GATE(X[3], 3)
+        WNWG_RUN(4, ps[5])
+        WNWG_GATE(X[4], 4)
+        WNWG_RUN(5, nch)
+        WNWG_DRAIN()
+        WNWG_GATE(X[5], 5)
     }
 #undef WNWG_DRAIN
 #undef WNWG_RUN
@@ -378,6 +414,11 @@
     return wn_winograd_layer_supported(C, H) && 4 * (C / GEMM_KC) + 2 * ((C + H) / GEMM_KC) + 2 * (H / GEMM_KC) <= WNWG_MAX_CHUNKS;
 }
 
+bool wn_winograd_layer_f63_supported(int C, int H) {
+    return wn_winograd_layer_f43_supported(C, H) && H % (2 * GEMM_KC) == 0 &&
+           6 * (C / GEMM_KC) + 2 * ((C + H) / GEMM_KC) + 4 * (H / GEMM_KC) <= WNWG_MAX_CHUNKS;
+}
+
 namespace {
 thread_local int t_last_f43_width = 0;
 
@@ -400,9 +441,11 @@
     WnWinogradLayerArgs a = a_in;
     CTTS_CHECK_ARG(wn_winograd_layer_supported(a.C, a.H), "wn_winograd_layer: C=%d H=%d", a.C, a.H);
     CTTS_CHECK_ARG(a.A_T2 && a.A_T3 && a.A_e && a.A_o && a.bias && a.V && a.act && a.batch >= 1, "wn_winograd_layer: operand not set");
-    const bool f43 = a.form == WNWG_F43;
-    const int tw = f43 ? 64 : 128;
-    CTTS_CHECK_ARG(a.form == WNWG_F23 || (f43 && wn_winograd_layer_f43_supported(a.C, a.H) && a.A_T4 && a.A_T5), "wn_winograd_layer: form %d", a.form);
+    const bool f43 = a.form == WNWG_F43, f63 = a.form == WNWG_F63;
+    const int tw = f43 || f63 ? 64 : 128;
+    CTTS_CHECK_ARG(a.form == WNWG_F23 || (f43 && wn_winograd_layer_f43_supported(a.C, a.H) && a.A_T4 && a.A_T5) ||
+                       (f63 && wn_winograd_layer_f63_supported(a.C, a.H) && a.A_T4 && a.A_T5 && a.A_T6 && a.A_T7 && a.in_place),
+                   "wn_winograd_layer: form %d", a.form);
     CTTS_CHECK_ARG(a.d >= 1 && a.L >= 1 && a.Lp >= 1 && a.ntiles >= 1 && a.Lp <= a.ntiles * tw && a.ntiles * tw <= a.ldp && a.ldp % 4 == 0 &&
                        a.ld % 4 == 0 && a.pad >= 0 && a.pad % 4 == 0 && a.L + a.pad <= a.ld,
                    "wn_winograd_layer: geometry d=%d L=%d Lp=%d ntiles=%d ldp=%d ld=%d pad=%d", a.d, a.L, a.Lp, a.ntiles, a.ldp, a.ld, a.pad);
@@ -412,6 +455,7 @@
     a.b0 = 0;
     a.col0 = 0;
     const Tuning tn = tuning();
+    if (f63) return launch_wnwg_shape<1, 2, 2, 1>(a, a.ntiles, (long long)a.ntiles * a.batch, stream);
     if (f43) {
         const bool kd2 = a.H % (2 * GEMM_KC) == 0;
         if (tn.f32_no_small && kd2) {
diff --git a/include/cookietts_hip.h b/include/cookietts_hip.h
--- a/include/cookietts_hip.h
+++ b/include/cookietts_hip.h
@@ -661,6 +661,7 @@
 
 int ctts_tuning_reload(void);
 int ctts_tuning_flags(void);
+int ctts_tuning_flags_ext(void);
 
 #define CTTS_PROF_WN_IN 0
 #define CTTS_PROF_WN_RS 1
```

Result: faster. 4.314 million samples/s, median of 6 (+6.0%).
